# uc-vision/taichi-splatting

Measured on AMD Instinct MI355X. Metric: fwd+bwd Msplats/s, higher is better.
Workload: dtype f32; 1 GPU; config D: 6000000 random 3D gaussians, 2048x2048, SH deg 3, tile 16, fwd+bwd (render_gaussians, loss=image.sum()); n_gaussians=6000000, tile_size=16, sh_degree=3, mode=single, parallelism=single GPU

## Files before the change

taichi_splatting_amd/csrc/frame.hip:

```cpp
#include <cstdlib>
#include <cstring>
#include "common.h"
#include "frame_internal.h"
#include "raster_common.h"

namespace ms {

struct FrameGeom {
  int w_pad, h_pad, tiles_wide, tiles_high, num_tiles, tile_bits, row_begin, row_end;
  size_t es;
};

static FrameGeom frame_geom(const ms_frame_desc* d) {
  FrameGeom g;
  const int ts = d->raster.tile_size;
  g.tiles_wide = (d->image_w + ts - 1) / ts;
  g.tiles_high = (d->image_h + ts - 1) / ts;
  g.w_pad = g.tiles_wide * ts;
  g.h_pad = g.tiles_high * ts;
  g.num_tiles = g.tiles_wide * g.tiles_high;
  int bits = 1;
  while ((1ll << bits) < (long long)g.num_tiles) ++bits;
  g.tile_bits = bits;
  g.row_begin = d->tile_row_begin < 0 ? 0 : d->tile_row_begin;
  g.row_end = d->tile_row_end > g.tiles_high ? g.tiles_high : d->tile_row_end;
  g.es = d->dtype == MS_F64 ? 8 : 4;
  return g;
}

static int check_desc(const ms_frame_desc* d, const char* who) {
  if (!d) { set_error("%s: desc is null", who); return MS_ERR_BAD_ARG; }
  if (d->struct_size != sizeof(ms_frame_desc) || MS_ABI_GENERATION(d->abi_version) != MS_ABI_GENERATION(MS_VERSION)) {
    set_error("%s: ms_frame_desc of another ABI (struct_size %u, abi_version %u; this library: %u, %d) — set desc.struct_size = "
              "sizeof(ms_frame_desc) and desc.abi_version = MS_VERSION of the include/mi355_splat.h you compile against",
              who, d->struct_size, d->abi_version, (unsigned)sizeof(ms_frame_desc), MS_VERSION);
    return MS_ERR_ABI;
  }
  if (d->split_long_runs < 0 || d->split_seg_len < 0) { set_error("%s: negative split parameter", who); return MS_ERR_BAD_ARG; }
  if (d->n < 0 || d->k_capacity < 0) { set_error("%s: negative size", who); return MS_ERR_BAD_ARG; }
  if (d->n >= (1ll << 31) || d->k_capacity >= (1ll << 31)) { set_error("%s: sizes are int32 indexes (< 2^31)", who); return MS_ERR_BAD_ARG; }
  if (d->image_w <= 0 || d->image_h <= 0) { set_error("%s: bad image size", who); return MS_ERR_BAD_ARG; }
  if (d->dtype != MS_F32 && d->dtype != MS_F64) { set_error("%s: dtype must be MS_F32 or MS_F64", who); return MS_ERR_BAD_ARG; }
  const int ts = d->raster.tile_size;
  if (ts != 8 && ts != 16 && ts != 32) { set_error("%s: tile_size must be 8, 16 or 32 (got %d)", who, ts); return MS_ERR_UNSUPPORTED; }
  if (d->f < 1 || d->f > 4) { set_error("%s: 1..4 colour channels (got %d)", who, d->f); return MS_ERR_UNSUPPORTED; }
  if (d->sh_degree < -1 || d->sh_degree > 3) { set_error("%s: SH degree must be in [0, 3]", who); return MS_ERR_BAD_ARG; }
  if (d->mapper != MS_MAPPER_DIRECT && d->mapper != MS_MAPPER_PRESORT) { set_error("%s: mapper must be MS_MAPPER_DIRECT or MS_MAPPER_PRESORT (got %d)", who, d->mapper); return MS_ERR_BAD_ARG; }
  if (d->projected_input && d->sh_degree >= 0) { set_error("%s: projected input carries colours, not SH", who); return MS_ERR_BAD_ARG; }
  if (d->depth16) {
    const FrameGeom g = frame_geom(d);
    if (g.num_tiles > 65536) { set_error("%s: use_depth16 keys hold a 16 bit tile id: too many tiles", who); return MS_ERR_BAD_ARG; }
  }
  return 0;
}

static bool frame_uses_rows(const ms_frame_desc* d) {
  static const bool on = [] { const char* e = getenv("MS_SPLAT_ROWS"); return e && e[0] == '1'; }();
  return on && !d->projected_input && d->n > 0 && raster_uses_splat_rows(&d->raster, d->f, d->dtype);
}

static bool frame_uses_split(const ms_frame_desc* d) {
  return d->split_long_runs != 0 && d->n > 0 && d->k_capacity > 0 && raster_uses_splat_rows(&d->raster, d->f, d->dtype);
}
static SplitParams frame_split_params(const ms_frame_desc* d) {
  return split_params(d->raster.tile_size, d->split_long_runs, d->split_seg_len);
}

static int check_inputs(const ms_frame_inputs* in, const char* who) {
  if (!in) { set_error("%s: inputs are null", who); return MS_ERR_BAD_ARG; }
  if (in->struct_size != sizeof(ms_frame_inputs)) {
    set_error("%s: ms_frame_inputs of another ABI (struct_size %u, this library: %u)", who, in->struct_size, (unsigned)sizeof(ms_frame_inputs));
    return MS_ERR_ABI;
  }
  return 0;
}

static int check_grads(const ms_frame_grads* g, const char* who) {
  if (!g) { set_error("%s: grads are null", who); return MS_ERR_BAD_ARG; }
  if (g->struct_size != sizeof(ms_frame_grads)) {
    set_error("%s: ms_frame_grads of another ABI (struct_size %u, this library: %u)", who, g->struct_size, (unsigned)sizeof(ms_frame_grads));
    return MS_ERR_ABI;
  }
  return 0;
}

struct Carve {
  size_t off = 0;
  size_t take(size_t bytes) { const size_t o = off; off += align_up(bytes > 0 ? bytes : 1, 256); return o; }
};

static void frame_layout(const ms_frame_desc* d, ms_frame_layout* L) {
  const FrameGeom g = frame_geom(d);
  const size_t n = (size_t)d->n, k = (size_t)d->k_capacity;
  const bool own_points = !d->projected_input;
  Carve keep_n, scratch_n, keep_k, scratch_k;
  L->points7 = keep_n.take(own_points ? n * 7 * g.es : 0);
  L->depth = keep_n.take(own_points ? n * g.es : 0);
  L->colours = keep_n.take(d->sh_degree >= 0 ? n * d->f * g.es : 0);
  L->camera_position = keep_n.take(4 * g.es);
  L->counters = keep_n.take(8 * sizeof(int32_t));
  L->tile_ranges = keep_n.take((size_t)g.num_tiles * 2 * sizeof(int32_t));
  L->splat_rows = keep_n.take(frame_uses_rows(d) ? n * SPLAT_ROW * sizeof(float) : 0);
  L->keep_n_bytes = keep_n.off;

  L->sorted_keys = scratch_n.take(n * 4);
  L->order = scratch_n.take(n * 4);
  L->counts = scratch_n.take(n * 4);
  L->cum = scratch_n.take((n + 1) * 4);
  L->ordered_points = scratch_n.take(n * 7 * 4);
  L->points7_f32 = scratch_n.take(d->dtype == MS_F64 ? n * 7 * 4 : 0);
  const size_t t1 = sort_tmp_size(d->n, 4, true), t2 = scan_tmp_size(d->n);
  L->tmp_n = scratch_n.take(t1 > t2 ? t1 : t2);
  L->scratch_n_bytes = scratch_n.off;

  L->overlap_to_point = keep_k.take(k * 4);
  L->split_scratch = keep_k.take(frame_uses_split(d) ? split_scratch_bytes(d->k_capacity, d->raster.tile_size, frame_split_params(d)) : 0);
  L->keep_k_bytes = keep_k.off;

  L->keys = scratch_k.take(k * 8);
  L->values = scratch_k.take(k * 4);
  L->keys_sorted = scratch_k.take(k * 8);
  L->tmp_k = scratch_k.take(sort_tmp_size(d->k_capacity, 8));
  L->scratch_k_bytes = scratch_k.off;
}

template <typename T>
__global__ void __launch_bounds__(256)
frame_prepare_kernel(int32_t* __restrict__ counters, int32_t capacity, const T* __restrict__ Tcw, T* __restrict__ cam_out,
                     int32_t* __restrict__ ranges, int64_t range_words) {
  const int64_t i = (int64_t)blockIdx.x * blockDim.x + threadIdx.x;
  if (i < range_words) ranges[i] = 0;
  if (i == 0) {
    const int32_t k = counters[0];
    const bool ok = k >= 0 && k <= capacity;
    counters[1] = ok ? k : 0;
    counters[2] = ok ? 0 : 1;
    counters[3] = 0;
    counters[4] = 0;
    counters[5] = 0;
    if (cam_out) camera_position_solve(Tcw, cam_out);
  }
}

__global__ void __launch_bounds__(256)
f64_to_f32_kernel(const double* __restrict__ in, float* __restrict__ out, int64_t count) {
  const int64_t i = (int64_t)blockIdx.x * blockDim.x + threadIdx.x;
  if (i < count) out[i] = (float)in[i];
}

static bool mapper_presort(const ms_frame_desc& d) {
  static const int forced = [] {
    const char* e = getenv("MS_MAPPER");
    if (e && strcmp(e, "presort") == 0) return MS_MAPPER_PRESORT;
    if (e && strcmp(e, "direct") == 0) return MS_MAPPER_DIRECT;
    return -1;
  }();
  return (forced >= 0 ? forced : d.mapper) == MS_MAPPER_PRESORT;
}

static bool frame_uses_moments(const ms_frame_desc* d, int deterministic) {
  (void)deterministic;
  return d->dtype == MS_F32 && d->f == 3 && !d->raster.antialias && d->raster.use_alpha_blending;
}

}

using namespace ms;

extern "C" int ms_frame_layout_query(const ms_frame_desc* desc, ms_frame_layout* out) {
  int rc = check_desc(desc, "ms_frame_layout_query");
  if (rc) return rc;
  MS_CHECK_ARG(out != nullptr, "out is null");
  frame_layout(desc, out);
  return 0;
}

extern "C" int ms_frame_uses_moments(const ms_frame_desc* desc, int deterministic) {
  return desc && frame_uses_moments(desc, deterministic) ? 1 : 0;
}

#define MS_TRY(expr)            \
  do {                          \
    const int rc__ = (expr);    \
    if (rc__ != 0) return rc__; \
  } while (0)

static int frame_project_impl(const ms_frame_desc* desc, const ms_frame_inputs* in, void* keep_n, bool projection,
                              bool colours, void* stream, const char* who) {
  const ms_frame_desc& d = *desc;
  if (d.projected_input) { set_error("%s: projected input has no per-gaussian stage", who); return MS_ERR_BAD_ARG; }
  if (d.n == 0) return 0;
  ms_frame_layout L;
  frame_layout(desc, &L);
  char* kn = (char*)keep_n;
  if (!(in->position && in->log_scaling && in->rotation && in->alpha_logit && in->T_camera_world && in->projection)) {
    set_error("%s: null gaussian / camera input", who); return MS_ERR_BAD_ARG;
  }
  if (!in->feature) { set_error("%s: feature is null", who); return MS_ERR_BAD_ARG; }
  float* rows = frame_uses_rows(desc) ? (float*)(kn + L.splat_rows) : nullptr;
  if (projection) {
    if (d.sh_degree >= 0 && colours)
      MS_TRY(ms_camera_position(in->T_camera_world, kn + L.camera_position, d.dtype, stream));
    MS_TRY(project_fwd_launch(in->position, in->log_scaling, in->rotation, in->alpha_logit, in->T_camera_world, in->projection,
                              d.image_w, d.image_h, d.near_plane, d.far_plane, d.blur_cov, d.clamp_margin,
                              d.raster.alpha_threshold, d.n, kn + L.points7, kn + L.depth, nullptr, d.dtype, stream, rows,
                              rows && d.sh_degree < 0 ? in->feature : nullptr));
  }
  if (colours && d.sh_degree >= 0)
    MS_TRY(sh_fwd_inplace_launch(in->feature, in->position, kn + L.depth, kn + L.camera_position, d.n, d.f,
                                 d.sh_degree, kn + L.colours, d.dtype, (hipStream_t)stream, rows));
  return 0;
}

extern "C" int ms_frame_project(const ms_frame_desc* desc, const ms_frame_inputs* in, void* keep_n, void* stream) {
  MS_TRY(check_desc(desc, "ms_frame_project"));
  MS_TRY(check_inputs(in, "ms_frame_project"));
  MS_CHECK_ARG(in && keep_n, "null pointer");
  return frame_project_impl(desc, in, keep_n, true, true, stream, "ms_frame_project");
}

extern "C" int ms_frame_sh_colours(const ms_frame_desc* desc, const ms_frame_inputs* in, void* keep_n, void* stream) {
  MS_TRY(check_desc(desc, "ms_frame_sh_colours"));
  MS_TRY(check_inputs(in, "ms_frame_sh_colours"));
  MS_CHECK_ARG(in && keep_n, "null pointer");
  const ms_frame_desc& d = *desc;
  MS_CHECK_ARG(!d.projected_input && d.sh_degree >= 0, "a frame that evaluates SH colours itself");
  MS_CHECK_ARG(!frame_uses_rows(desc), "the splat-row table is filled on the frame's own stream");
  if (d.n == 0) return 0;
  ms_frame_layout L;
  frame_layout(desc, &L);
  MS_CHECK_ARG(in->T_camera_world != nullptr, "T_camera_world is null");
  MS_TRY(ms_camera_position(in->T_camera_world, (char*)keep_n + L.camera_position, d.dtype, stream));
  return frame_project_impl(desc, in, keep_n, false, true, stream, "ms_frame_sh_colours");
}

extern "C" int ms_frame_project_count(const ms_frame_desc* desc, const ms_frame_inputs* in, void* keep_n,
                                      void* scratch_n, int32_t* k_host, void* k_event, void* stream) {
  MS_TRY(check_desc(desc, "ms_frame_project_count"));
  MS_TRY(check_inputs(in, "ms_frame_project_count"));
  MS_CHECK_ARG(in && keep_n && scratch_n, "null pointer");
  const ms_frame_desc& d = *desc;
  const FrameGeom g = frame_geom(desc);
  ms_frame_layout L;
  frame_layout(desc, &L);
  hipStream_t s = (hipStream_t)stream;
  char* kn = (char*)keep_n;
  char* sn = (char*)scratch_n;
  int32_t* counters = (int32_t*)(kn + L.counters);

  if (d.n == 0) {
    MS_CHECK_HIP(hipMemsetAsync(counters, 0, 8 * sizeof(int32_t), s));
    if (k_host) *k_host = 0;
    if (k_event) MS_CHECK_HIP(hipEventRecord((hipEvent_t)k_event, s));
    return 0;
  }

  const void* points7;
  const void* depth;
  if (!d.projected_input) {
    MS_TRY(frame_project_impl(desc, in, keep_n, true, false, stream, "ms_frame_project_count"));
    points7 = kn + L.points7;
    depth = kn + L.depth;
  } else {
    MS_CHECK_ARG(in->points7 && in->depth && in->colours, "null projected input");
    points7 = in->points7;
    depth = in->depth;
  }

  const float* points_f32 = (const float*)points7;
  if (d.dtype == MS_F64) {
    float* copy = (float*)(sn + L.points7_f32);
    f64_to_f32_kernel<<<dim3((unsigned)div_up(d.n * 7, 256)), dim3(256), 0, s>>>((const double*)points7, copy, d.n * 7);
    points_f32 = copy;
  }

  uint32_t* sorted_keys = (uint32_t*)(sn + L.sorted_keys);
  int32_t* order = (int32_t*)(sn + L.order);
  int32_t* counts = (int32_t*)(sn + L.counts);
  int32_t* cum = (int32_t*)(sn + L.cum);
  const int cull = d.projected_input ? 0 : 1;
  if (mapper_presort(d)) {
    depth_argsort_launch(depth, d.n, d.depth16, d.near_plane > 0.0 ? d.near_plane : 0.0, d.far_plane, d.dtype, cull,
                         sorted_keys, order, sn + L.tmp_n, s);
    tile_count_launch(points_f32, order, cull ? sorted_keys : nullptr, d.n, g.w_pad, g.h_pad, d.raster.tile_size,
                      (float)d.raster.alpha_threshold, g.row_begin, g.row_end, counts, (float*)(sn + L.ordered_points), s);
  } else {
    tile_count_direct_launch(points_f32, cull ? depth : nullptr, d.dtype, d.n, g.w_pad, g.h_pad, d.raster.tile_size,
                             (float)d.raster.alpha_threshold, g.row_begin, g.row_end, counts, s);
  }
  exclusive_scan_launch(counts, d.n, cum, k_host, sn + L.tmp_n, s, counters);
  MS_CHECK_LAUNCH();
  if (k_event) MS_CHECK_HIP(hipEventRecord((hipEvent_t)k_event, s));
  return 0;
}

extern "C" int ms_frame_map_raster(const ms_frame_desc* desc, const ms_frame_inputs* in, void* keep_n, void* scratch_n,
                                   void* keep_k, void* scratch_k, void* out_image, void* out_alpha,
                                   void* out_visibility, void* stream) {
  MS_TRY(check_desc(desc, "ms_frame_map_raster"));
  MS_TRY(check_inputs(in, "ms_frame_map_raster"));
  MS_CHECK_ARG(in && keep_n && scratch_n && out_image && out_alpha, "null pointer");
  const ms_frame_desc& d = *desc;
  const FrameGeom g = frame_geom(desc);
  ms_frame_layout L;
  frame_layout(desc, &L);
  hipStream_t s = (hipStream_t)stream;
  char* kn = (char*)keep_n;
  char* sn = (char*)scratch_n;
  char* kk = (char*)keep_k;
  char* sk = (char*)scratch_k;
  int32_t* counters = (int32_t*)(kn + L.counters);
  int32_t* ranges = (int32_t*)(kn + L.tile_ranges);
  int32_t* o2p = (int32_t*)(kk + L.overlap_to_point);
  const bool colours_elsewhere = !d.projected_input && d.sh_degree >= 0 && in->colours_ready_event != nullptr;

  {
    const bool want_cam = !d.projected_input && d.sh_degree >= 0 && d.n > 0 && !colours_elsewhere;
    if (want_cam) MS_CHECK_ARG(in->T_camera_world != nullptr, "T_camera_world is null");
    const int64_t words = (int64_t)g.num_tiles * 2;
    const dim3 grid((unsigned)(words > 0 ? div_up(words, 256) : 1)), block(256);
    if (d.dtype == MS_F64)
      frame_prepare_kernel<double><<<grid, block, 0, s>>>(counters, (int32_t)d.k_capacity, (const double*)in->T_camera_world,
                                                          want_cam ? (double*)(kn + L.camera_position) : nullptr, ranges, words);
    else
      frame_prepare_kernel<float><<<grid, block, 0, s>>>(counters, (int32_t)d.k_capacity, (const float*)in->T_camera_world,
                                                         want_cam ? (float*)(kn + L.camera_position) : nullptr, ranges, words);
  }
  if (!d.projected_input && !colours_elsewhere) MS_TRY(frame_project_impl(desc, in, keep_n, false, true, stream, "ms_frame_map_raster"));
  if (d.n > 0 && d.k_capacity > 0) {
    MS_CHECK_ARG(keep_k && scratch_k, "null overlap buffers");
    int32_t* values = (int32_t*)(sk + L.values);
    if (mapper_presort(d)) {
      uint32_t* keys = (uint32_t*)(sk + L.keys);
      uint32_t* keys_sorted = (uint32_t*)(sk + L.keys_sorted);
      tile_emit_ordered_launch((const float*)(sn + L.ordered_points), (const int32_t*)(sn + L.order),
                               (const int32_t*)(sn + L.cum), d.n, g.w_pad, g.h_pad, d.raster.tile_size,
                               (float)d.raster.alpha_threshold, g.row_begin, g.row_end, counters + 1, keys, values, s);
      sort_pairs_u32_dev_launch(keys, values, keys_sorted, o2p, d.k_capacity, counters + 1, g.tile_bits, sk + L.tmp_k, s);
      MS_TRY(find_ranges_dev_launch(keys_sorted, d.k_capacity, counters + 1, g.num_tiles, ranges, s, true));
    } else {
      uint64_t* keys = (uint64_t*)(sk + L.keys);
      uint64_t* keys_sorted = (uint64_t*)(sk + L.keys_sorted);
      const void* depth = d.projected_input ? in->depth : (const void*)(kn + L.depth);
      const float* points_f32 = d.dtype == MS_F64 ? (const float*)(sn + L.points7_f32)
                                                  : (const float*)(d.projected_input ? in->points7 : (const void*)(kn + L.points7));
      tile_emit_direct_launch(points_f32, depth, d.dtype, (const int32_t*)(sn + L.cum), d.n, g.w_pad, g.h_pad,
                              d.raster.tile_size, (float)d.raster.alpha_threshold, g.row_begin, g.row_end, d.depth16,
                              d.near_plane > 0.0 ? d.near_plane : 0.0, d.far_plane, counters + 1, keys, values, s);
      sort_pairs_u64_dev_launch(keys, values, keys_sorted, o2p, d.k_capacity, counters + 1, 32, 32 + g.tile_bits,
                                sk + L.tmp_k, s);
      MS_TRY(find_ranges_u64_dev_launch(keys_sorted, d.k_capacity, counters + 1, g.num_tiles, ranges, s));
      const int64_t first_tile = (int64_t)g.row_begin * g.tiles_wide;
      const int64_t strip_tiles = (int64_t)(g.row_end > g.row_begin ? g.row_end - g.row_begin : 0) * g.tiles_wide;
      tile_depth_sort_launch(ranges + 2 * first_tile, strip_tiles, keys_sorted, o2p, keys, s, counters + 3, in->longest_run_host);
    }
  }
  MS_CHECK_LAUNCH();

  const void* points7 = d.projected_input ? in->points7 : (const void*)(kn + L.points7);
  const void* colours = d.sh_degree >= 0 ? (const void*)(kn + L.colours) : (d.projected_input ? in->colours : in->feature);
  MS_CHECK_ARG(d.n == 0 || colours != nullptr, "colours are null");
  SplitScratch split{};
  const bool cut = frame_uses_split(desc) && keep_k != nullptr;
  if (cut) split = split_scratch_carve(kk + L.split_scratch, d.k_capacity, d.raster.tile_size, frame_split_params(desc));
  if (in->colours_ready_event) MS_CHECK_HIP(hipStreamWaitEvent(s, (hipEvent_t)in->colours_ready_event, 0));
  return raster_fwd_launch(points7, colours, frame_uses_rows(desc) ? (const float*)(kn + L.splat_rows) : nullptr, ranges, o2p,
                           d.image_w, d.image_h, d.f, &d.raster, out_image, out_alpha, out_visibility, g.row_begin, g.row_end,
                           d.dtype, stream, cut ? &split : nullptr, in->longest_run_host);
}

extern "C" int ms_frame_backward(const ms_frame_desc* desc, const ms_frame_inputs* in, void* keep_n, void* keep_k,
                                 const ms_frame_grads* gr, void* stream) {
  MS_TRY(check_desc(desc, "ms_frame_backward"));
  MS_TRY(check_inputs(in, "ms_frame_backward"));
  MS_TRY(check_grads(gr, "ms_frame_backward"));
  MS_CHECK_ARG(in && keep_n && gr, "null pointer");
  MS_CHECK_ARG(gr->stage == MS_BACKWARD_GAUSSIANS || (gr->image && gr->grad_image), "null image / grad_image");
  const ms_frame_desc& d = *desc;
  const FrameGeom g = frame_geom(desc);
  ms_frame_layout L;
  frame_layout(desc, &L);
  hipStream_t s = (hipStream_t)stream;
  char* kn = (char*)keep_n;
  char* kk = (char*)keep_k;
  const int32_t* ranges = (const int32_t*)(kn + L.tile_ranges);
  const int32_t* o2p = (const int32_t*)(kk + L.overlap_to_point);
  const void* points7 = d.projected_input ? in->points7 : (const void*)(kn + L.points7);
  const void* depth = d.projected_input ? in->depth : (const void*)(kn + L.depth);
  const void* colours = d.sh_degree >= 0 ? (const void*)(kn + L.colours) : (d.projected_input ? in->colours : in->feature);
  if (d.n == 0) return 0;

  const bool given = gr->stage == MS_BACKWARD_GAUSSIANS;
  const bool raster_only = gr->stage == MS_BACKWARD_RASTER || d.projected_input;
  const bool moments = !given && frame_uses_moments(desc, gr->deterministic);
  MS_CHECK_ARG(!gr->grad_image_broadcast || (!given && moments), "grad_image_broadcast: moments path only (float32 RGB, plain pdf)");
  MS_CHECK_ARG(gr->boundary_form == MS_BOUNDARY_AXIS_SIGMA || gr->boundary_form == MS_BOUNDARY_COVARIANCE, "boundary_form");
  MS_CHECK_ARG(gr->boundary_form == 0 || given || (moments && gr->stage == MS_BACKWARD_RASTER),
               "MS_BOUNDARY_COVARIANCE rows: MS_BACKWARD_GAUSSIANS, or MS_BACKWARD_RASTER on the moments path");
  if (gr->boundary_stride != 0) {
    MS_CHECK_ARG(gr->boundary_stride >= 7 + d.f && d.dtype == MS_F32, "boundary_stride: rows of >= 7 + f floats, float32 frames");
    MS_CHECK_ARG(given || (moments && raster_only), "boundary_stride: MS_BACKWARD_GAUSSIANS, or MS_BACKWARD_RASTER on the moments path");
  }
  if (given) {
    MS_CHECK_ARG(!d.projected_input, "projected input has no per-gaussian backward");
    if (gr->gather_world > 0)
      MS_CHECK_ARG(gr->gather_rows && gr->gather_slots && gr->gather_route && gr->boundary_stride >= 7 + d.f && d.dtype == MS_F32,
                   "gathered boundary gradients: rows, slots, route, boundary_stride >= 7 + f, float32");
    else
      MS_CHECK_ARG(gr->grad_points7 != nullptr, "grad_points7 is null");
  } else if (moments) {
    MS_CHECK_ARG(gr->moments != nullptr, "moments is null");
    SplitScratch split{};
    const bool cut = frame_uses_split(desc) && keep_k != nullptr;
    if (cut) split = split_scratch_carve(kk + L.split_scratch, d.k_capacity, d.raster.tile_size, frame_split_params(desc));
    MS_TRY(raster_bwd_moments_launch(points7, colours, ranges, o2p, gr->image, gr->grad_image, d.image_w, d.image_h, &d.raster,
                                     (float*)gr->moments, gr->deterministic, gr->fixed_exp, g.row_begin, g.row_end,
                                     gr->grad_image_broadcast, s,
                                     frame_uses_rows(desc) ? (const float*)(kn + L.splat_rows) : nullptr,
                                     cut ? &split : nullptr));
    if (raster_only)
      return moments_finalize_rezero_launch((const float*)points7, (float*)gr->moments, gr->deterministic, gr->fixed_exp,
                                            d.n, (float*)gr->grad_points7, (float*)gr->grad_colours,
                                            d.raster.compute_point_heuristic ? (float*)gr->point_heuristic : nullptr, s,
                                            gr->boundary_stride, d.projected_input && gr->stage != MS_BACKWARD_RASTER ? 0 : gr->boundary_form);
  } else {
    MS_CHECK_ARG(gr->grad_points7 || gr->grad_colours, "no gradient accumulator");
    MS_TRY(ms_raster_bwd(points7, colours, ranges, o2p, gr->image, gr->grad_image, d.image_w, d.image_h, d.f, &d.raster,
                         gr->grad_points7, gr->grad_colours, d.raster.compute_point_heuristic ? gr->point_heuristic : nullptr,
                         g.row_begin, g.row_end, d.dtype, stream));
    if (raster_only) return 0;
  }

  GaussianBwdArgs a{};
  a.dtype = d.dtype;
  a.n = d.n;
  a.position = in->position; a.log_scaling = in->log_scaling; a.rotation = in->rotation; a.alpha_logit = in->alpha_logit;
  a.T_camera_world = in->T_camera_world; a.projection = in->projection;
  a.image_w = d.image_w; a.image_h = d.image_h;
  a.blur_cov = d.blur_cov; a.clamp_margin = d.clamp_margin;
  a.depth = depth;
  if (moments) {
    a.moments = gr->moments; a.deterministic = gr->deterministic; a.fixed_exp = gr->fixed_exp;
    a.store_points7 = gr->grad_points7; a.store_colours = gr->grad_colours;
    a.point_heuristic = d.raster.compute_point_heuristic ? gr->point_heuristic : nullptr;
    a.point_visibility = d.raster.compute_point_heuristic ? gr->point_visibility : nullptr;
  } else {
    a.grad_points7 = gr->grad_points7; a.grad_colours = gr->grad_colours;
    a.boundary_stride = gr->boundary_stride;
    a.boundary_cov = given ? gr->boundary_form : 0;
    if (given && gr->gather_world > 0) {
      a.gather_world = gr->gather_world; a.gather_rows = gr->gather_rows;
      a.gather_slots = gr->gather_slots; a.gather_route = gr->gather_route;
    }
  }
  a.extra_points7 = gr->extra_points7; a.extra_depth = gr->extra_depth; a.extra_colours = gr->extra_colours;
  a.sh_degree = d.sh_degree; a.f = d.f;
  a.camera_position = kn + L.camera_position; a.colours = colours;
  a.grad_position = gr->grad_position; a.grad_log_scaling = gr->grad_log_scaling; a.grad_rotation = gr->grad_rotation;
  a.grad_alpha_logit = gr->grad_alpha_logit; a.grad_feature = gr->grad_feature; a.grad_camera = gr->grad_camera;
  return gaussian_bwd_launch(a, s);
}
```

taichi_splatting_amd/csrc/frame_internal.h:

```cpp
#pragma once
#include "common.h"

namespace ms {

constexpr uint32_t CULLED_DEPTH_KEY = 0xffffffffu;

template <typename T>
__device__ inline void camera_position_solve(const T* __restrict__ m, T* __restrict__ out) {
#pragma clang fp contract(off)
  double a[4][5];
  for (int r = 0; r < 4; ++r) {
    for (int c = 0; c < 4; ++c) a[r][c] = (double)m[r * 4 + c];
    a[r][4] = r == 3 ? 1.0 : 0.0;
  }
  for (int col = 0; col < 4; ++col) {
    int piv = col;
    for (int r = col + 1; r < 4; ++r)
      if (fabs(a[r][col]) > fabs(a[piv][col])) piv = r;
    for (int c = 0; c < 5; ++c) { const double t = a[col][c]; a[col][c] = a[piv][c]; a[piv][c] = t; }
    const double inv = 1.0 / a[col][col];
    for (int c = 0; c < 5; ++c) a[col][c] *= inv;
    for (int r = 0; r < 4; ++r) {
      if (r == col) continue;
      const double fct = a[r][col];
      for (int c = 0; c < 5; ++c) a[r][c] -= fct * a[col][c];
    }
  }
  for (int k = 0; k < 3; ++k) out[k] = (T)a[k][4];
}

size_t scan_tmp_size(int64_t n);
size_t sort_tmp_size(int64_t n, int key_bytes, bool adaptive = false);
void exclusive_scan_launch(const int32_t* in, int64_t n, int32_t* out, int32_t* total_host, void* tmp, hipStream_t s,
                           int32_t* total_copy = nullptr);
void depth_argsort_launch(const void* depth, int64_t n, int depth16, double ndc_near, double ndc_far, int dtype,
                          int cull, uint32_t* out_sorted_keys, int32_t* out_order, char* tmp, hipStream_t s);
void sort_pairs_u32_dev_launch(const uint32_t* keys_in, const int32_t* vals_in, uint32_t* keys_out, int32_t* vals_out,
                               int64_t capacity, const int32_t* n_dev, int end_bit, char* tmp, hipStream_t s);
int find_ranges_dev_launch(const uint32_t* sorted_keys, int64_t capacity, const int32_t* k_dev, int64_t num_tiles,
                           int32_t* out_ranges, hipStream_t s, bool zeroed = false);

void sort_pairs_u64_dev_launch(const uint64_t* keys_in, const int32_t* vals_in, uint64_t* keys_out, int32_t* vals_out,
                               int64_t capacity, const int32_t* n_dev, int begin_bit, int end_bit, char* tmp, hipStream_t s);
int find_ranges_u64_dev_launch(const uint64_t* sorted_keys, int64_t capacity, const int32_t* k_dev, int64_t num_tiles,
                               int32_t* out_ranges, hipStream_t s);

void tile_count_launch(const float* points7, const int32_t* order, const uint32_t* cull_keys, int64_t v, int image_w,
                       int image_h, int tile_size, float alpha_threshold, int row_begin, int row_end,
                       int32_t* out_counts, float* out_ordered, hipStream_t s);
void tile_emit_ordered_launch(const float* ordered_points7, const int32_t* order, const int32_t* cum, int64_t v,
                              int image_w, int image_h, int tile_size, float alpha_threshold, int row_begin,
                              int row_end, const int32_t* k_limit_dev, uint32_t* out_keys, int32_t* out_values,
                              hipStream_t s);

void tile_count_direct_launch(const float* points7, const void* cull_depth, int dtype, int64_t v, int image_w, int image_h,
                              int tile_size, float alpha_threshold, int row_begin, int row_end, int32_t* out_counts,
                              hipStream_t s);
void tile_emit_direct_launch(const float* points7, const void* depth, int dtype, const int32_t* cum, int64_t v, int image_w,
                             int image_h, int tile_size, float alpha_threshold, int row_begin, int row_end, int depth16,
                             double ndc_near, double ndc_far, const int32_t* k_limit_dev, uint64_t* out_keys,
                             int32_t* out_values, hipStream_t s);

void tile_depth_sort_launch(const int32_t* tile_ranges, int64_t num_tiles, uint64_t* sorted_keys, int32_t* overlap_to_point,
                            uint64_t* scratch, hipStream_t s, int32_t* run_stats = nullptr, int32_t* run_host = nullptr);

int project_fwd_launch(const void* position, const void* log_scaling, const void* rotation, const void* alpha_logit,
                       const void* T_camera_world, const void* projection, int image_w, int image_h, double near_plane,
                       double far_plane, double blur_cov, double clamp_margin, double alpha_threshold, int64_t n,
                       void* out_points7, void* out_depth, int32_t* out_flag, int dtype, void* stream, float* splat_rows,
                       const void* colours_in);

int sh_fwd_inplace_launch(const void* params, const void* positions, const void* depth, const void* cam_pos,
                          int64_t n, int f, int degree, void* out, int dtype, hipStream_t s, float* splat_rows = nullptr);

bool raster_uses_splat_rows(const ms_raster_config* cfg, int f, int dtype);
int raster_fwd_launch(const void* points7, const void* features, const float* splat_rows, const int32_t* tile_ranges,
                      const int32_t* overlap_to_point, int image_w, int image_h, int f, const ms_raster_config* cfg,
                      void* out_image, void* out_alpha, void* out_visibility, int tile_row_begin, int tile_row_end,
                      int dtype, void* stream, const struct SplitScratch* split = nullptr, int32_t* long_run_word = nullptr);

int raster_bwd_moments_launch(const void* points7, const void* features, const int32_t* tile_ranges,
                              const int32_t* overlap_to_point, const void* image, const void* grad_image, int image_w,
                              int image_h, const ms_raster_config* cfg, float* moments, int deterministic,
                              const int32_t* fixed_exp, int tile_row_begin, int tile_row_end, int grad_broadcast,
                              hipStream_t s, const float* splat_rows = nullptr, const struct SplitScratch* split = nullptr);
int moments_finalize_rezero_launch(const float* points7, float* moments, int deterministic, const int32_t* fixed_exp,
                                   int64_t n, float* grad_points7, float* grad_features, float* point_heuristic,
                                   hipStream_t s, int row_stride = 0, int covariance_form = 0);

struct GaussianBwdArgs {
  int dtype;
  int64_t n;
  const void *position, *log_scaling, *rotation, *alpha_logit, *T_camera_world, *projection;
  int image_w, image_h;
  double blur_cov, clamp_margin;
  const void* depth;
  void* moments;
  int deterministic;
  const int32_t* fixed_exp;
  const void* grad_points7;
  const void* grad_colours;
  int boundary_cov;
  int boundary_stride;
  int gather_world;
  const void* gather_rows;
  const int32_t *gather_slots, *gather_route;
  const void *extra_points7, *extra_depth, *extra_colours;
  int sh_degree, f;
  const void *camera_position, *colours;
  void *grad_position, *grad_log_scaling, *grad_rotation, *grad_alpha_logit;
  void* grad_feature;
  void* grad_camera;
  void *store_points7, *store_colours;
  void* point_heuristic;
  void* point_visibility;
};
int gaussian_bwd_launch(const GaussianBwdArgs& a, hipStream_t s);

}
```

taichi_splatting_amd/csrc/mapper.hip:

```cpp
#pragma clang fp contract(off)
#include "common.h"
#include "frame_internal.h"

namespace ms {

__device__ __forceinline__ void load_point7(const float* __restrict__ points, int64_t i, float g[7]) {
#pragma unroll
  for (int k = 0; k < 7; ++k) g[k] = points[i * 7 + k];
}


__device__ __forceinline__ float readlane_f(float v, int lane) {
  return __int_as_float(__builtin_amdgcn_readlane(__float_as_int(v), lane));
}
__device__ __forceinline__ ObbQuery wave_broadcast(const ObbQuery& q, int lane) {
  ObbQuery r;
  r.inv00 = readlane_f(q.inv00, lane); r.inv01 = readlane_f(q.inv01, lane);
  r.inv10 = readlane_f(q.inv10, lane); r.inv11 = readlane_f(q.inv11, lane);
  r.rel_min_x = readlane_f(q.rel_min_x, lane); r.rel_min_y = readlane_f(q.rel_min_y, lane);
  r.min_tile_x = __builtin_amdgcn_readlane(q.min_tile_x, lane); r.min_tile_y = __builtin_amdgcn_readlane(q.min_tile_y, lane);
  r.span_x = __builtin_amdgcn_readlane(q.span_x, lane); r.span_y = __builtin_amdgcn_readlane(q.span_y, lane);
  return r;
}
__device__ __forceinline__ unsigned long long wide_span_lanes(const ObbQuery& q, bool valid, int* my_span) {
  const int span = valid && q.span_x > 0 && q.span_y > 0 ? q.span_x * q.span_y : 0;
  *my_span = span;
  const int total = (int)readlane_f(wave_sum_to_lane63((float)span), 63);
  int thr = total / 32;
  thr = thr > 16 ? thr : 16;
  return __ballot(span > thr);
}
template <typename F>
__device__ __forceinline__ void wave_walk_span(const ObbQuery& b, int tile_size, int row_begin, int row_end, F on_hits) {
  const int n = b.span_x * b.span_y, lane = lane_id();
  for (int base = 0; base < n; base += 64) {
    const int idx = base + lane;
    bool hit = false;
    int tu = 0, tv = 0;
    if (idx < n) {
      tv = idx / b.span_x; tu = idx - tv * b.span_x;
      const int ty = b.min_tile_y + tv;
      hit = ty >= row_begin && ty < row_end && obb_test_tile(b, tu, tv, tile_size);
    }
    on_hits(hit, b.min_tile_x + tu, b.min_tile_y + tv);
  }
}
__device__ __forceinline__ int count_span(const ObbQuery& q, bool valid, int tile_size, int row_begin, int row_end) {
  int span;
  unsigned long long wide = wide_span_lanes(q, valid, &span);
  const bool mine_is_wide = (wide >> lane_id()) & 1ull;
  int count = 0;
  if (span > 0 && !mine_is_wide) {
    for (int tv = 0; tv < q.span_y; ++tv) {
      const int ty = q.min_tile_y + tv;
      if (ty < row_begin || ty >= row_end) continue;
      for (int tu = 0; tu < q.span_x; ++tu)
        if (obb_test_tile(q, tu, tv, tile_size)) ++count;
    }
  }
  while (wide != 0) {
    const int src = __builtin_ctzll(wide);
    wide &= wide - 1;
    const ObbQuery b = wave_broadcast(q, src);
    int total = 0;
    wave_walk_span(b, tile_size, row_begin, row_end, [&](bool hit, int, int) { total += __builtin_popcountll(__ballot(hit)); });
    if (lane_id() == src) count = total;
  }
  return count;
}
template <typename F>
__device__ __forceinline__ void emit_span(const ObbQuery& q, bool valid, int64_t first, int tile_size, int row_begin,
                                          int row_end, F emit) {
  int span;
  unsigned long long wide = wide_span_lanes(q, valid, &span);
  const bool mine_is_wide = (wide >> lane_id()) & 1ull;
  if (span > 0 && !mine_is_wide) {
    int64_t o = first;
    for (int tu = 0; tu < q.span_x; ++tu) {
      for (int tv = 0; tv < q.span_y; ++tv) {
        const int ty = q.min_tile_y + tv;
        if (ty < row_begin || ty >= row_end) continue;
        if (obb_test_tile(q, tu, tv, tile_size)) emit(o++, q.min_tile_x + tu, ty, -1);
      }
    }
  }
  while (wide != 0) {
    const int src = __builtin_ctzll(wide);
    wide &= wide - 1;
    const ObbQuery b = wave_broadcast(q, src);
    const int lo = __builtin_amdgcn_readlane((int)(uint32_t)first, src), hi = __builtin_amdgcn_readlane((int)(uint32_t)(first >> 32), src);
    int64_t o = (int64_t)(((uint64_t)(uint32_t)hi << 32) | (uint32_t)lo);
    wave_walk_span(b, tile_size, row_begin, row_end, [&](bool hit, int tx, int ty) {
      const unsigned long long m = __ballot(hit);
      if (hit) emit(o + (int)__builtin_amdgcn_mbcnt_hi((uint32_t)(m >> 32), __builtin_amdgcn_mbcnt_lo((uint32_t)m, 0u)), tx, ty, src);
      o += __builtin_popcountll(m);
    });
  }
}

__global__ void __launch_bounds__(256)
tile_count_kernel(const float* __restrict__ points, const int32_t* __restrict__ order,
                  const uint32_t* __restrict__ cull_keys, int64_t v, int image_w,
                  int image_h, int tile_size, float alpha_threshold, int row_begin, int row_end,
                  int32_t* __restrict__ counts, float* __restrict__ ordered_points) {
  const int64_t i = (int64_t)blockIdx.x * blockDim.x + threadIdx.x;
  const bool valid = i < v && !(cull_keys && cull_keys[i] == CULLED_DEPTH_KEY);
  float g[7] = {0.f, 0.f, 1.f, 0.f, 1.f, 1.f, 0.f};
  if (valid) {
    load_point7(points, order ? (int64_t)order[i] : i, g);
    if (ordered_points) {
#pragma unroll
      for (int k = 0; k < 7; ++k) ordered_points[i * 7 + k] = g[k];
    }
  }
  const ObbQuery q = obb_grid_query(g, image_w, image_h, tile_size, alpha_threshold);
  const int count = count_span(q, valid, tile_size, row_begin, row_end);
  if (i < v) counts[i] = count;
}

template <typename KeyT, int MODE>
__global__ void __launch_bounds__(256)
tile_emit_kernel(const float* __restrict__ points, const float* __restrict__ depth,
                 const int32_t* __restrict__ order, const int32_t* __restrict__ cum, int64_t v,
                 int image_w, int image_h, int tile_size, float alpha_threshold, int row_begin,
                 int row_end, int points_ordered, const int32_t* __restrict__ k_limit,
                 KeyT* __restrict__ keys, int32_t* __restrict__ values) {
  const int64_t i = (int64_t)blockIdx.x * blockDim.x + threadIdx.x;
  if (k_limit && *k_limit == 0) return;
  const bool valid = i < v && !(k_limit && cum[i + 1] == cum[i]);
  const int64_t src = valid ? (order ? (int64_t)order[i] : i) : 0;
  float g[7] = {0.f, 0.f, 1.f, 0.f, 1.f, 1.f, 0.f};
  if (valid) load_point7(points, points_ordered ? i : src, g);
  const ObbQuery q = obb_grid_query(g, image_w, image_h, tile_size, alpha_threshold);
  const int tiles_wide = image_w / tile_size;
  KeyT depth_key = 0;
  if (valid) {
    if (MODE == 1) {
      const float c = fminf(fmaxf(depth[src], 0.0f), 1.0f);
      depth_key = (KeyT)(uint32_t)(c * 65535.0f);
    } else if (MODE == 0) {
      depth_key = (KeyT)__float_as_uint(depth[src]);
    }
  }
  const uint32_t dk_lo = (uint32_t)depth_key, dk_hi = (uint32_t)((uint64_t)depth_key >> 32);
  emit_span(q, valid, valid ? (int64_t)cum[i] : 0, tile_size, row_begin, row_end, [&](int64_t o, int tx, int ty, int from) {
    const int64_t tile_id = (int64_t)tx + (int64_t)ty * tiles_wide;
    KeyT dk = depth_key;
    int32_t who = (int32_t)src;
    if (from >= 0) {
      dk = (KeyT)(((uint64_t)(uint32_t)__builtin_amdgcn_readlane((int)dk_hi, from) << 32) | (uint32_t)__builtin_amdgcn_readlane((int)dk_lo, from));
      who = __builtin_amdgcn_readlane((int32_t)src, from);
    }
    if constexpr (MODE == 2) keys[o] = (KeyT)tile_id;
    else if constexpr (MODE == 1) keys[o] = (KeyT)(dk | ((KeyT)tile_id << 16));
    else keys[o] = (KeyT)(dk | ((KeyT)tile_id << 32));
    values[o] = who;
  });
}

template <typename T>
__global__ void __launch_bounds__(256, 8)
tile_count_direct_kernel(const float* __restrict__ points, const T* __restrict__ cull_depth, int64_t v, int image_w,
                         int image_h, int tile_size, float alpha_threshold, int row_begin, int row_end,
                         int32_t* __restrict__ counts) {
  const int64_t i = (int64_t)blockIdx.x * blockDim.x + threadIdx.x;
  const bool valid = i < v && !(cull_depth && !(cull_depth[i] > T(0)));
  float g[7] = {0.f, 0.f, 1.f, 0.f, 1.f, 1.f, 0.f};
  if (valid) load_point7(points, i, g);
  const ObbQuery q = obb_grid_query(g, image_w, image_h, tile_size, alpha_threshold);
  const int count = count_span(q, valid, tile_size, row_begin, row_end);
  if (i < v) counts[i] = count;
}

template <typename T>
__global__ void __launch_bounds__(256)
tile_emit_direct_kernel(const float* __restrict__ points, const T* __restrict__ depth, const int32_t* __restrict__ cum,
                        int64_t v, int image_w, int image_h, int tile_size, float alpha_threshold, int row_begin,
                        int row_end, int depth16, double near_plane, double far_plane,
                        const int32_t* __restrict__ k_limit, uint64_t* __restrict__ keys, int32_t* __restrict__ values) {
  const int64_t i = (int64_t)blockIdx.x * blockDim.x + threadIdx.x;
  if (k_limit && *k_limit == 0) return;
  const int64_t first = i < v ? (int64_t)cum[i] : 0;
  const bool valid = i < v && cum[i + 1] != first;
  float g[7] = {0.f, 0.f, 1.f, 0.f, 1.f, 1.f, 0.f};
  if (valid) load_point7(points, i, g);
  const ObbQuery q = obb_grid_query(g, image_w, image_h, tile_size, alpha_threshold);
  const int tiles_wide = image_w / tile_size;
  const uint32_t depth_key = valid ? (uint32_t)depth_sort_key(depth[i], depth16, near_plane, far_plane) : 0u;
  emit_span(q, valid, first, tile_size, row_begin, row_end, [&](int64_t o, int tx, int ty, int from) {
    const uint64_t tile_id = (uint64_t)((int64_t)tx + (int64_t)ty * tiles_wide);
    uint32_t dk = depth_key;
    int32_t who = (int32_t)i;
    if (from >= 0) { dk = (uint32_t)__builtin_amdgcn_readlane((int)depth_key, from); who = __builtin_amdgcn_readlane((int32_t)i, from); }
    keys[o] = (tile_id << 32) | dk;
    values[o] = who;
  });
}

template <typename T>
__global__ void __launch_bounds__(256)
depth_keys_kernel(const T* __restrict__ depth, int64_t v, int depth16, double near_plane, double far_plane,
                  uint32_t* __restrict__ keys, int32_t* __restrict__ values) {
  const int64_t i = (int64_t)blockIdx.x * blockDim.x + threadIdx.x;
  if (i >= v) return;
  keys[i] = depth_sort_key(depth[i], depth16, near_plane, far_plane);
  values[i] = (int32_t)i;
}

void tile_count_launch(const float* points7, const int32_t* order, const uint32_t* cull_keys, int64_t v, int image_w,
                       int image_h, int tile_size, float alpha_threshold, int row_begin, int row_end,
                       int32_t* out_counts, float* out_ordered, hipStream_t s) {
  tile_count_kernel<<<dim3((unsigned)div_up(v, 256)), dim3(256), 0, s>>>(
      points7, order, cull_keys, v, image_w, image_h, tile_size, alpha_threshold, row_begin, row_end, out_counts, out_ordered);
}

void tile_emit_ordered_launch(const float* ordered_points7, const int32_t* order, const int32_t* cum, int64_t v,
                              int image_w, int image_h, int tile_size, float alpha_threshold, int row_begin,
                              int row_end, const int32_t* k_limit_dev, uint32_t* out_keys, int32_t* out_values,
                              hipStream_t s) {
  tile_emit_kernel<uint32_t, 2><<<dim3((unsigned)div_up(v, 256)), dim3(256), 0, s>>>(
      ordered_points7, nullptr, order, cum, v, image_w, image_h, tile_size, alpha_threshold, row_begin, row_end, 1,
      k_limit_dev, out_keys, out_values);
}

void tile_count_direct_launch(const float* points7, const void* cull_depth, int dtype, int64_t v, int image_w, int image_h,
                              int tile_size, float alpha_threshold, int row_begin, int row_end, int32_t* out_counts,
                              hipStream_t s) {
  const dim3 grid((unsigned)div_up(v, 256)), block(256);
  if (dtype == MS_F64)
    tile_count_direct_kernel<double><<<grid, block, 0, s>>>(points7, (const double*)cull_depth, v, image_w, image_h, tile_size,
                                                            alpha_threshold, row_begin, row_end, out_counts);
  else
    tile_count_direct_kernel<float><<<grid, block, 0, s>>>(points7, (const float*)cull_depth, v, image_w, image_h, tile_size,
                                                           alpha_threshold, row_begin, row_end, out_counts);
}

void tile_emit_direct_launch(const float* points7, const void* depth, int dtype, const int32_t* cum, int64_t v, int image_w,
                             int image_h, int tile_size, float alpha_threshold, int row_begin, int row_end, int depth16,
                             double ndc_near, double ndc_far, const int32_t* k_limit_dev, uint64_t* out_keys,
                             int32_t* out_values, hipStream_t s) {
  const dim3 grid((unsigned)div_up(v, 256)), block(256);
  if (dtype == MS_F64)
    tile_emit_direct_kernel<double><<<grid, block, 0, s>>>(points7, (const double*)depth, cum, v, image_w, image_h, tile_size,
                                                           alpha_threshold, row_begin, row_end, depth16, ndc_near, ndc_far,
                                                           k_limit_dev, out_keys, out_values);
  else
    tile_emit_direct_kernel<float><<<grid, block, 0, s>>>(points7, (const float*)depth, cum, v, image_w, image_h, tile_size,
                                                          alpha_threshold, row_begin, row_end, depth16, ndc_near, ndc_far,
                                                          k_limit_dev, out_keys, out_values);
}

}

using namespace ms;

extern "C" int ms_depth_sort_keys(const void* depth, int64_t v, int depth16, double ndc_near, double ndc_far,
                                  uint32_t* out_keys, int32_t* out_values, int dtype, void* stream) {
  MS_CHECK_ARG(v >= 0, "v < 0");
  MS_CHECK_ARG(dtype == MS_F32 || dtype == MS_F64, "dtype must be MS_F32 or MS_F64");
  if (v == 0) return 0;
  MS_CHECK_ARG(depth && out_keys && out_values, "null pointer");
  const dim3 grid((unsigned)div_up(v, 256)), block(256);
  if (dtype == MS_F32)
    depth_keys_kernel<float><<<grid, block, 0, (hipStream_t)stream>>>((const float*)depth, v, depth16, ndc_near, ndc_far, out_keys, out_values);
  else
    depth_keys_kernel<double><<<grid, block, 0, (hipStream_t)stream>>>((const double*)depth, v, depth16, ndc_near, ndc_far, out_keys, out_values);
  MS_CHECK_LAUNCH();
  return 0;
}

extern "C" int ms_tile_count(const float* points7, const int32_t* order, int64_t v, int image_w, int image_h, int tile_size,
                             float alpha_threshold, int tile_row_begin, int tile_row_end,
                             int32_t* out_counts, float* out_ordered_points7, void* stream) {
  MS_CHECK_ARG(v >= 0, "v < 0");
  MS_CHECK_ARG(tile_size > 0 && image_w > 0 && image_h > 0, "bad image/tile size");
  MS_CHECK_ARG(image_w % tile_size == 0 && image_h % tile_size == 0, "image size must be padded to the tile size");
  if (v == 0) return 0;
  MS_CHECK_ARG(points7 && out_counts, "null pointer");
  tile_count_kernel<<<dim3((unsigned)div_up(v, 256)), dim3(256), 0, (hipStream_t)stream>>>(
      points7, order, nullptr, v, image_w, image_h, tile_size, alpha_threshold, tile_row_begin, tile_row_end, out_counts, out_ordered_points7);
  MS_CHECK_LAUNCH();
  return 0;
}

extern "C" int ms_tile_emit(const float* points7, const float* depth, const int32_t* order, const int32_t* cum,
                            int64_t v, int image_w, int image_h, int tile_size, float alpha_threshold,
                            int tile_row_begin, int tile_row_end, int key_mode, int points_are_ordered,
                            void* out_keys, int32_t* out_values, void* stream) {
  MS_CHECK_ARG(v >= 0, "v < 0");
  MS_CHECK_ARG(key_mode >= 0 && key_mode <= 2, "key_mode must be 0 (tile|depth32), 1 (tile|depth16) or 2 (tile only)");
  MS_CHECK_ARG(tile_size > 0 && image_w > 0 && image_h > 0, "bad image/tile size");
  MS_CHECK_ARG(image_w % tile_size == 0 && image_h % tile_size == 0, "image size must be padded to the tile size");
  if (key_mode == 1) {
    const int64_t tiles = (int64_t)(image_w / tile_size) * (image_h / tile_size);
    MS_CHECK_ARG(tiles <= 65536, "use_depth16 keys hold a 16 bit tile id: too many tiles");
  }
  if (v == 0) return 0;
  MS_CHECK_ARG(points7 && cum && out_keys && out_values, "null pointer");
  MS_CHECK_ARG(key_mode == 2 || depth, "depth is null");
  const dim3 block(256), grid((unsigned)div_up(v, 256));
  hipStream_t s = (hipStream_t)stream;
#define MS_EMIT(KeyT, MODE) tile_emit_kernel<KeyT, MODE><<<grid, block, 0, s>>>(points7, depth, order, cum, v, image_w, image_h, tile_size, alpha_threshold, tile_row_begin, tile_row_end, points_are_ordered, nullptr, (KeyT*)out_keys, out_values)
  if (key_mode == 0) MS_EMIT(uint64_t, 0);
  else if (key_mode == 1) MS_EMIT(uint32_t, 1);
  else MS_EMIT(uint32_t, 2);
#undef MS_EMIT
  MS_CHECK_LAUNCH();
  return 0;
}

extern "C" int ms_tile_emit_keys64(const float* points7, const void* depth, int depth_dtype, const int32_t* cum, int64_t v,
                                   int image_w, int image_h, int tile_size, float alpha_threshold, int tile_row_begin,
                                   int tile_row_end, int depth16, double ndc_near, double ndc_far, uint64_t* out_keys,
                                   int32_t* out_values, void* stream) {
  MS_CHECK_ARG(v >= 0, "v < 0");
  MS_CHECK_ARG(depth_dtype == MS_F32 || depth_dtype == MS_F64, "depth_dtype must be MS_F32 or MS_F64");
  MS_CHECK_ARG(tile_size > 0 && image_w > 0 && image_h > 0, "bad image/tile size");
  MS_CHECK_ARG(image_w % tile_size == 0 && image_h % tile_size == 0, "image size must be padded to the tile size");
  if (depth16) {
    const int64_t tiles = (int64_t)(image_w / tile_size) * (image_h / tile_size);
    MS_CHECK_ARG(tiles <= 65536, "use_depth16 keys hold a 16 bit tile id: too many tiles");
  }
  if (v == 0) return 0;
  MS_CHECK_ARG(points7 && depth && cum && out_keys && out_values, "null pointer");
  tile_emit_direct_launch(points7, depth, depth_dtype, cum, v, image_w, image_h, tile_size, alpha_threshold, tile_row_begin,
                          tile_row_end, depth16, ndc_near > 0.0 ? ndc_near : 0.0, ndc_far, nullptr, out_keys, out_values,
                          (hipStream_t)stream);
  MS_CHECK_LAUNCH();
  return 0;
}
```

taichi_splatting_amd/csrc/scan_sort.hip:

```cpp
#include "common.h"
#include "frame_internal.h"

namespace ms {

constexpr int SCAN_THREADS = 256;
constexpr int SCAN_ITEMS = 16;
constexpr int SCAN_TILE = SCAN_THREADS * SCAN_ITEMS;

__device__ __forceinline__ int block_exclusive_scan(int v, int* lds , int* block_total) {
  const int lane = lane_id(), wave = threadIdx.x >> 6;
  int incl = v;
#pragma unroll
  for (int off = 1; off < 64; off <<= 1) {
    const int t = __shfl_up(incl, off, 64);
    if (lane >= off) incl += t;
  }
  if (lane == 63) lds[wave] = incl;
  __syncthreads();
  int wave_off = 0, total = 0;
#pragma unroll
  for (int w = 0; w < SCAN_THREADS / 64; ++w) {
    const int s = lds[w];
    if (w < wave) wave_off += s;
    total += s;
  }
  __syncthreads();
  *block_total = total;
  return wave_off + incl - v;
}

__device__ __forceinline__ void load_items(const int32_t* __restrict__ in, int64_t base, int64_t n, int (&vals)[SCAN_ITEMS]) {
  if (base + SCAN_ITEMS <= n && (reinterpret_cast<uintptr_t>(in + base) & 15) == 0) {
    const int4* p = reinterpret_cast<const int4*>(in + base);
#pragma unroll
    for (int q = 0; q < SCAN_ITEMS / 4; ++q) {
      const int4 v = p[q];
      vals[4 * q] = v.x; vals[4 * q + 1] = v.y; vals[4 * q + 2] = v.z; vals[4 * q + 3] = v.w;
    }
  } else {
#pragma unroll
    for (int k = 0; k < SCAN_ITEMS; ++k) vals[k] = base + k < n ? in[base + k] : 0;
  }
}

__device__ __forceinline__ void store_items(int32_t* __restrict__ out, int64_t base, int64_t n, const int (&vals)[SCAN_ITEMS]) {
  if (base + SCAN_ITEMS <= n && (reinterpret_cast<uintptr_t>(out + base) & 15) == 0) {
    int4* p = reinterpret_cast<int4*>(out + base);
#pragma unroll
    for (int q = 0; q < SCAN_ITEMS / 4; ++q) p[q] = make_int4(vals[4 * q], vals[4 * q + 1], vals[4 * q + 2], vals[4 * q + 3]);
  } else {
#pragma unroll
    for (int k = 0; k < SCAN_ITEMS; ++k) if (base + k < n) out[base + k] = vals[k];
  }
}

__global__ void __launch_bounds__(SCAN_THREADS)
scan_block_sums_kernel(const int32_t* __restrict__ in, int64_t n, int32_t* __restrict__ block_sums) {
  __shared__ int lds[4];
  const int64_t base = (int64_t)blockIdx.x * SCAN_TILE + (int64_t)threadIdx.x * SCAN_ITEMS;
  int items[SCAN_ITEMS];
  load_items(in, base, n, items);
  int s = 0;
#pragma unroll
  for (int k = 0; k < SCAN_ITEMS; ++k) s += items[k];
  int total;
  block_exclusive_scan(s, lds, &total);
  if (threadIdx.x == 0) block_sums[blockIdx.x] = total;
}

__global__ void __launch_bounds__(SCAN_THREADS)
scan_spine_kernel(int32_t* __restrict__ block_sums, int64_t num_blocks, int32_t* __restrict__ total_out,
                  int32_t* __restrict__ total_host, int32_t* __restrict__ total_copy = nullptr) {
  __shared__ int lds[4];
  int carry = 0;
  for (int64_t base = 0; base < num_blocks; base += SCAN_THREADS) {
    const int64_t i = base + threadIdx.x;
    const int v = i < num_blocks ? block_sums[i] : 0;
    int total;
    const int ex = block_exclusive_scan(v, lds, &total);
    if (i < num_blocks) block_sums[i] = carry + ex;
    carry += total;
  }
  if (threadIdx.x == 0) {
    *total_out = carry;
    if (total_copy) *total_copy = carry;
    if (total_host) *total_host = carry;
  }
}

__global__ void __launch_bounds__(SCAN_THREADS)
scan_downsweep_kernel(const int32_t* __restrict__ in, int64_t n, const int32_t* __restrict__ block_offsets,
                      int32_t* __restrict__ out) {
  __shared__ int lds[4];
  const int64_t base = (int64_t)blockIdx.x * SCAN_TILE + (int64_t)threadIdx.x * SCAN_ITEMS;
  int vals[SCAN_ITEMS];
  load_items(in, base, n, vals);
  int s = 0;
#pragma unroll
  for (int k = 0; k < SCAN_ITEMS; ++k) s += vals[k];
  int total;
  int prefix = block_exclusive_scan(s, lds, &total) + block_offsets[blockIdx.x];
#pragma unroll
  for (int k = 0; k < SCAN_ITEMS; ++k) {
    const int v = vals[k];
    vals[k] = prefix;
    prefix += v;
  }
  store_items(out, base, n, vals);
}

constexpr int64_t SCAN_SELF_MAX_BLOCKS = 8192;

__global__ void __launch_bounds__(SCAN_THREADS)
scan_downsweep_self_kernel(const int32_t* __restrict__ in, int64_t n, const int32_t* __restrict__ block_sums,
                           int32_t* __restrict__ out, int32_t* __restrict__ total_host,
                           int32_t* __restrict__ total_copy = nullptr) {
  __shared__ int lds[4];
  int before = 0;
  for (int j = threadIdx.x; j < (int)blockIdx.x; j += SCAN_THREADS) before += block_sums[j];
  int block_prefix;
  block_exclusive_scan(before, lds, &block_prefix);

  const int64_t base = (int64_t)blockIdx.x * SCAN_TILE + (int64_t)threadIdx.x * SCAN_ITEMS;
  int vals[SCAN_ITEMS];
  load_items(in, base, n, vals);
  int s = 0;
#pragma unroll
  for (int k = 0; k < SCAN_ITEMS; ++k) s += vals[k];
  int total;
  int prefix = block_exclusive_scan(s, lds, &total) + block_prefix;
#pragma unroll
  for (int k = 0; k < SCAN_ITEMS; ++k) {
    const int v = vals[k];
    vals[k] = prefix;
    prefix += v;
  }
  store_items(out, base, n, vals);
  if (blockIdx.x == gridDim.x - 1 && threadIdx.x == 0) {
    out[n] = block_prefix + total;
    if (total_copy) *total_copy = block_prefix + total;
    if (total_host) *total_host = block_prefix + total;
  }
}

static size_t scan_tmp_bytes(int64_t n) { return align_up((size_t)div_up(n > 0 ? n : 1, SCAN_TILE) * sizeof(int32_t), 256); }

static int exclusive_scan_i32(const int32_t* in, int64_t n, int32_t* out, int32_t* total_host, void* tmp,
                              hipStream_t s, int32_t* total_copy = nullptr) {
  const int64_t blocks = div_up(n, SCAN_TILE);
  int32_t* block_sums = (int32_t*)tmp;
  scan_block_sums_kernel<<<dim3((unsigned)blocks), dim3(SCAN_THREADS), 0, s>>>(in, n, block_sums);
  if (blocks <= SCAN_SELF_MAX_BLOCKS) {
    scan_downsweep_self_kernel<<<dim3((unsigned)blocks), dim3(SCAN_THREADS), 0, s>>>(in, n, block_sums, out, total_host, total_copy);
    return 0;
  }
  scan_spine_kernel<<<dim3(1), dim3(SCAN_THREADS), 0, s>>>(block_sums, blocks, out + n, total_host, total_copy);
  scan_downsweep_kernel<<<dim3((unsigned)blocks), dim3(SCAN_THREADS), 0, s>>>(in, n, block_sums, out);
  return 0;
}

constexpr int RS_THREADS = 256;
constexpr int RS_WAVES = RS_THREADS / 64;
constexpr int RS_ROUNDS = 16;
constexpr int RS_WAVE_ITEMS = RS_ROUNDS * 64;
constexpr int RS_TILE = RS_THREADS * RS_ROUNDS;
constexpr int RS_RADIX = 256;

template <typename KeyT>
__device__ __forceinline__ unsigned key_digit(KeyT k, int shift, unsigned mask) {
  return (unsigned)(k >> shift) & mask;
}

template <typename KeyT> struct PlainPairs {
  const KeyT* keys;
  const int32_t* vals;
  __device__ __forceinline__ KeyT key(int64_t i) const { return keys[i]; }
  __device__ __forceinline__ int32_t val(int64_t i) const { return vals[i]; }
};
template <typename T> struct DepthPairs {
  const T* depth;
  int depth16;
  double near_plane, far_plane;
  int cull;
  __device__ __forceinline__ uint32_t key(int64_t i) const {
    const T d = depth[i];
    if (cull && !(d > T(0))) return CULLED_DEPTH_KEY;
    return depth_sort_key(d, depth16, near_plane, far_plane);
  }
  __device__ __forceinline__ int32_t val(int64_t i) const { return (int32_t)i; }
};

template <typename KeyT, typename Source, bool VARY = false>
__device__ __forceinline__ void upsweep_block(const Source src, int64_t n, int shift, unsigned mask,
                                              int32_t* __restrict__ hist, int64_t num_blocks,
                                              uint32_t* __restrict__ blk_or = nullptr, uint32_t* __restrict__ blk_and = nullptr) {
  constexpr int RS_COPIES = 4;
  __shared__ unsigned cnt[RS_WAVES][RS_COPIES][RS_RADIX];
  __shared__ unsigned s_or, s_and;
  for (int i = threadIdx.x; i < RS_WAVES * RS_COPIES * RS_RADIX; i += RS_THREADS) (&cnt[0][0][0])[i] = 0;
  if (VARY && threadIdx.x == 0) { s_or = 0u; s_and = ~0u; }
  __syncthreads();
  const int wave = threadIdx.x >> 6, lane = lane_id();
  unsigned* mine = cnt[wave][lane & (RS_COPIES - 1)];
  const int64_t base = (int64_t)blockIdx.x * RS_TILE + (int64_t)wave * RS_WAVE_ITEMS + lane;
  unsigned v_or = 0u, v_and = ~0u;
  if ((int64_t)(blockIdx.x + 1) * RS_TILE <= n) {
    KeyT k[RS_ROUNDS];
#pragma unroll
    for (int j = 0; j < RS_ROUNDS; ++j) k[j] = src.key(base + j * 64);
#pragma unroll
    for (int j = 0; j < RS_ROUNDS; ++j) {
      atomicAdd(&mine[key_digit(k[j], shift, mask)], 1u);
      if (VARY && (uint32_t)k[j] != 0xffffffffu) { v_or |= (uint32_t)k[j]; v_and &= (uint32_t)k[j]; }
    }
  } else {
#pragma unroll 4
    for (int j = 0; j < RS_ROUNDS; ++j) {
      const int64_t i = base + j * 64;
      if (i < n) {
        const KeyT key = src.key(i);
        atomicAdd(&mine[key_digit(key, shift, mask)], 1u);
        if (VARY && (uint32_t)key != 0xffffffffu) { v_or |= (uint32_t)key; v_and &= (uint32_t)key; }
      }
    }
  }
  if (VARY) {
#pragma unroll
    for (int off = 32; off >= 1; off >>= 1) { v_or |= __shfl_xor(v_or, off); v_and &= __shfl_xor(v_and, off); }
    if (lane == 0) { atomicOr(&s_or, v_or); atomicAnd(&s_and, v_and); }
  }
  __syncthreads();
  for (int d = threadIdx.x; d < RS_RADIX; d += RS_THREADS) {
    unsigned t = 0;
#pragma unroll
    for (int w = 0; w < RS_WAVES; ++w)
#pragma unroll
      for (int c = 0; c < RS_COPIES; ++c) t += cnt[w][c][d];
    hist[(int64_t)d * num_blocks + blockIdx.x] = (int32_t)t;
  }
  if (VARY && threadIdx.x == 0) { blk_or[blockIdx.x] = s_or; blk_and[blockIdx.x] = s_and; }
}

template <typename KeyT, typename Source>
__global__ void __launch_bounds__(RS_THREADS)
radix_upsweep_kernel(const Source src, int64_t n, const int32_t* __restrict__ n_dev, int shift, unsigned mask,
                     int32_t* __restrict__ hist, int64_t num_blocks) {
  if (n_dev) n = *n_dev;
  upsweep_block<KeyT, Source>(src, n, shift, mask, hist, num_blocks);
}

__device__ __forceinline__ void row_scan_body(int32_t* __restrict__ hist, int64_t num_blocks, int32_t* __restrict__ digit_totals) {
  __shared__ int lds[4];
  int32_t* row = hist + (int64_t)blockIdx.x * num_blocks;
  int carry = 0;
  for (int64_t base = 0; base < num_blocks; base += SCAN_TILE) {
    const int64_t mine = base + (int64_t)threadIdx.x * SCAN_ITEMS;
    int vals[SCAN_ITEMS];
    load_items(row, mine, num_blocks, vals);
    int s = 0;
#pragma unroll
    for (int k = 0; k < SCAN_ITEMS; ++k) s += vals[k];
    int total;
    int prefix = carry + block_exclusive_scan(s, lds, &total);
#pragma unroll
    for (int k = 0; k < SCAN_ITEMS; ++k) {
      const int v = vals[k];
      vals[k] = prefix;
      prefix += v;
    }
    store_items(row, mine, num_blocks, vals);
    carry += total;
  }
  if (threadIdx.x == 0) digit_totals[blockIdx.x] = carry;
}

__global__ void __launch_bounds__(SCAN_THREADS)
radix_row_scan_kernel(int32_t* __restrict__ hist, int64_t num_blocks, int32_t* __restrict__ digit_totals) {
  row_scan_body(hist, num_blocks, digit_totals);
}

template <typename KeyT> struct DownsweepShared {
  unsigned cnt[RS_WAVES][RS_RADIX];
  int scan[4];
  unsigned digit_shift[RS_RADIX];
  KeyT keys[RS_TILE];
  int32_t vals[RS_TILE];
};

template <typename KeyT, bool FULL, typename Source>
__device__ __forceinline__ void downsweep_block(DownsweepShared<KeyT>& sh, const Source src, KeyT* __restrict__ keys_out,
                                                int32_t* __restrict__ vals_out, int64_t n, int shift, unsigned mask,
                                                const int32_t* __restrict__ hist_scanned,
                                                const int32_t* __restrict__ digit_totals, int64_t num_blocks) {
  for (int i = threadIdx.x; i < RS_WAVES * RS_RADIX; i += RS_THREADS) (&sh.cnt[0][0])[i] = 0;
  __syncthreads();

  const int wave = threadIdx.x >> 6, lane = lane_id();
  const int64_t base = (int64_t)blockIdx.x * RS_TILE + (int64_t)wave * RS_WAVE_ITEMS + lane;
  const unsigned long long lanes_below = (1ull << lane) - 1ull;

  KeyT k[RS_ROUNDS];
  int32_t v[RS_ROUNDS];
  unsigned rank[RS_ROUNDS];

#pragma unroll
  for (int j = 0; j < RS_ROUNDS; ++j) {
    const int64_t i = base + j * 64;
    const bool valid = FULL || i < n;
    k[j] = valid ? src.key(i) : (KeyT)0;
    v[j] = valid ? src.val(i) : 0;
  }

#pragma unroll
  for (int j = 0; j < RS_ROUNDS; ++j) {
    const int64_t i = base + j * 64;
    const bool valid = FULL || i < n;
    const unsigned d = key_digit(k[j], shift, mask);
    const unsigned long long valid_lanes = FULL ? ~0ull : __ballot(valid);
    unsigned peers_lo = (unsigned)valid_lanes, peers_hi = (unsigned)(valid_lanes >> 32);
#pragma unroll
    for (int b = 0; b < 8; ++b) {
      const int m = __builtin_amdgcn_sbfe((int)d, b, 1);
      const unsigned long long bal = __ballot(m != 0);
      peers_lo &= ~((unsigned)bal ^ (unsigned)m);
      peers_hi &= ~((unsigned)(bal >> 32) ^ (unsigned)m);
    }
    const unsigned long long peers = ((unsigned long long)peers_hi << 32) | peers_lo;
    const unsigned below = (unsigned)__popcll(peers & lanes_below);
    unsigned prev = 0;
    if (valid) {
      prev = sh.cnt[wave][d];
    }
    __builtin_amdgcn_wave_barrier();
    if (valid && below == 0) sh.cnt[wave][d] = prev + (unsigned)__popcll(peers);
    __builtin_amdgcn_wave_barrier();
    rank[j] = prev + below;
  }
  __syncthreads();

  {
    const int d = threadIdx.x;
    unsigned total = 0;
#pragma unroll
    for (int w = 0; w < RS_WAVES; ++w) total += sh.cnt[w][d];
    int block_total;
    const unsigned local = (unsigned)block_exclusive_scan((int)total, sh.scan, &block_total);
    unsigned run = local;
#pragma unroll
    for (int w = 0; w < RS_WAVES; ++w) {
      const unsigned c = sh.cnt[w][d];
      sh.cnt[w][d] = run;
      run += c;
    }
    int all_items;
    const unsigned digit_base = (unsigned)block_exclusive_scan(digit_totals[d], sh.scan, &all_items);
    sh.digit_shift[d] = digit_base + (unsigned)hist_scanned[(int64_t)d * num_blocks + blockIdx.x] - local;
  }
  __syncthreads();

#pragma unroll
  for (int j = 0; j < RS_ROUNDS; ++j) {
    const int64_t i = base + j * 64;
    if (FULL || i < n) {
      const unsigned d = key_digit(k[j], shift, mask);
      const unsigned lp = sh.cnt[wave][d] + rank[j];
      sh.keys[lp] = k[j];
      sh.vals[lp] = v[j];
    }
  }
  __syncthreads();
  const int64_t block_base = (int64_t)blockIdx.x * RS_TILE;
  const int block_items = FULL ? RS_TILE : (int)(n - block_base);
#pragma unroll
  for (int j = 0; j < RS_ROUNDS; ++j) {
    const int idx = (int)threadIdx.x + j * RS_THREADS;
    if (FULL || idx < block_items) {
      const KeyT key = sh.keys[idx];
      const unsigned d = key_digit(key, shift, mask);
      const int64_t pos = (int64_t)(unsigned)(sh.digit_shift[d] + (unsigned)idx);
      keys_out[pos] = key;
      vals_out[pos] = sh.vals[idx];
    }
  }
}

template <typename KeyT, typename Source>
__global__ void __launch_bounds__(RS_THREADS)
radix_downsweep_kernel(const Source src,
                       KeyT* __restrict__ keys_out, int32_t* __restrict__ vals_out, int64_t n,
                       const int32_t* __restrict__ n_dev, int shift,
                       unsigned mask, const int32_t* __restrict__ hist_scanned,
                       const int32_t* __restrict__ digit_totals, int64_t num_blocks) {
  __shared__ DownsweepShared<KeyT> sh;
  if (n_dev) {
    n = *n_dev;
    if ((int64_t)blockIdx.x * RS_TILE >= n) return;
  }
  if ((int64_t)(blockIdx.x + 1) * RS_TILE <= n)
    downsweep_block<KeyT, true>(sh, src, keys_out, vals_out, n, shift, mask, hist_scanned, digit_totals, num_blocks);
  else
    downsweep_block<KeyT, false>(sh, src, keys_out, vals_out, n, shift, mask, hist_scanned, digit_totals, num_blocks);
}

template <typename KeyT>
__global__ void __launch_bounds__(256)
copy_pairs_kernel(const KeyT* __restrict__ ki, const int32_t* __restrict__ vi, KeyT* __restrict__ ko,
                  int32_t* __restrict__ vo, int64_t n) {
  const int64_t i = (int64_t)blockIdx.x * blockDim.x + threadIdx.x;
  if (i < n) { ko[i] = ki[i]; vo[i] = vi[i]; }
}

struct SortTmp {
  size_t hist_off, scan_off, keys_off, vals_off, keys2_off, vals2_off, vary_off, total;
};

static SortTmp sort_tmp_layout(int64_t n, int key_bytes, bool adaptive = false) {
  const int64_t blocks = div_up(n > 0 ? n : 1, RS_TILE);
  SortTmp t;
  size_t off = 0;
  t.hist_off = off; off += align_up((size_t)(RS_RADIX * blocks + 1) * sizeof(int32_t), 256);
  t.scan_off = off; off += align_up((size_t)RS_RADIX * sizeof(int32_t), 256);
  t.keys_off = off; off += align_up((size_t)n * key_bytes, 256);
  t.vals_off = off; off += align_up((size_t)n * sizeof(int32_t), 256);
  t.keys2_off = t.vals2_off = t.vary_off = off;
  if (adaptive) {
    t.keys2_off = off; off += align_up((size_t)n * key_bytes, 256);
    t.vals2_off = off; off += align_up((size_t)n * sizeof(int32_t), 256);
    t.vary_off = off; off += align_up((size_t)(64 + 2 * blocks) * sizeof(uint32_t), 256);
  }
  t.total = off;
  return t;
}

template <typename KeyT, typename First>
static int radix_sort_passes(const First first, KeyT* keys_out, int32_t* vals_out, int64_t n, int begin_bit, int end_bit,
                             char* tmp, hipStream_t s, const int32_t* n_dev = nullptr) {
  const int64_t blocks = div_up(n, RS_TILE);
  const SortTmp lay = sort_tmp_layout(n, sizeof(KeyT));
  int32_t* hist = (int32_t*)(tmp + lay.hist_off);
  int32_t* digit_totals = (int32_t*)(tmp + lay.scan_off);
  KeyT* keys_alt = (KeyT*)(tmp + lay.keys_off);
  int32_t* vals_alt = (int32_t*)(tmp + lay.vals_off);
  const int passes = (end_bit - begin_bit + 7) / 8;
  const dim3 grid((unsigned)blocks), block(RS_THREADS);
  PlainPairs<KeyT> src{nullptr, nullptr};
  const int total_bits = end_bit - begin_bit, base_bits = total_bits / passes, wide = total_bits % passes;
  int shift = begin_bit;
  for (int p = 0; p < passes; shift += base_bits + (p < wide ? 1 : 0), ++p) {
    const int bits = base_bits + (p < wide ? 1 : 0);
    const unsigned mask = (1u << bits) - 1u;
    const bool to_out = ((passes - 1 - p) % 2) == 0;
    KeyT* dst_k = to_out ? keys_out : keys_alt;
    int32_t* dst_v = to_out ? vals_out : vals_alt;
    if (p == 0) radix_upsweep_kernel<KeyT, First><<<grid, block, 0, s>>>(first, n, n_dev, shift, mask, hist, blocks);
    else radix_upsweep_kernel<KeyT, PlainPairs<KeyT>><<<grid, block, 0, s>>>(src, n, n_dev, shift, mask, hist, blocks);
    radix_row_scan_kernel<<<dim3(RS_RADIX), dim3(SCAN_THREADS), 0, s>>>(hist, blocks, digit_totals);
    if (p == 0) radix_downsweep_kernel<KeyT, First><<<grid, block, 0, s>>>(first, dst_k, dst_v, n, n_dev, shift, mask, hist, digit_totals, blocks);
    else radix_downsweep_kernel<KeyT, PlainPairs<KeyT>><<<grid, block, 0, s>>>(src, dst_k, dst_v, n, n_dev, shift, mask, hist, digit_totals, blocks);
    src = PlainPairs<KeyT>{dst_k, dst_v};
  }
  return 0;
}

struct AdaptiveBufs {
  uint32_t *k_alt[2], *k_out;
  int32_t *v_alt[2], *v_out;
  uint32_t* vary;
};

__device__ __forceinline__ void adaptive_route(uint32_t vary, int p, int passes, bool& active, int& k, bool& last) {
  unsigned m = 1u;
  for (int q = 1; q < passes; ++q)
    if ((vary >> (8 * q)) & 0xffu) m |= 1u << q;
  active = ((m >> p) & 1u) != 0u;
  k = __popc(m & ((1u << p) - 1u));
  last = (m >> (p + 1)) == 0u;
}

template <typename First>
__global__ void __launch_bounds__(RS_THREADS)
depth_upsweep_first_kernel(const First first, AdaptiveBufs b, int64_t n, int32_t* __restrict__ hist, int64_t num_blocks) {
  upsweep_block<uint32_t, First, true>(first, n, 0, 0xffu, hist, num_blocks, b.vary + 64, b.vary + 64 + num_blocks);
}

__global__ void __launch_bounds__(RS_THREADS)
depth_upsweep_kernel(AdaptiveBufs b, int p, int passes, int64_t n, int32_t* __restrict__ hist, int64_t num_blocks) {
  bool active, last; int k;
  adaptive_route(b.vary[0], p, passes, active, k, last);
  if (!active) return;
  upsweep_block<uint32_t, PlainPairs<uint32_t>>(PlainPairs<uint32_t>{b.k_alt[(k - 1) & 1], b.v_alt[(k - 1) & 1]}, n, 8 * p, 0xffu, hist, num_blocks);
}

__global__ void __launch_bounds__(SCAN_THREADS)
depth_row_scan_kernel(int32_t* __restrict__ hist, int64_t num_blocks, int32_t* __restrict__ digit_totals, AdaptiveBufs b,
                      int p, int passes) {
  if (p > 0) {
    bool active, last; int k;
    adaptive_route(b.vary[0], p, passes, active, k, last);
    if (!active) return;
  }
  row_scan_body(hist, num_blocks, digit_totals);
  if (p == 0 && blockIdx.x == 0) {
    __shared__ unsigned s_or, s_and;
    if (threadIdx.x == 0) { s_or = 0u; s_and = ~0u; }
    __syncthreads();
    unsigned v_or = 0u, v_and = ~0u;
    for (int64_t i = threadIdx.x; i < num_blocks; i += blockDim.x) { v_or |= b.vary[64 + i]; v_and &= b.vary[64 + num_blocks + i]; }
    atomicOr(&s_or, v_or); atomicAnd(&s_and, v_and);
    __syncthreads();
    if (threadIdx.x == 0) b.vary[0] = s_or >= s_and && s_or != 0u ? (s_or ^ s_and) : 0u;
  }
}

template <typename First>
__global__ void __launch_bounds__(RS_THREADS)
depth_downsweep_first_kernel(const First first, AdaptiveBufs b, int passes, int64_t n,
                             const int32_t* __restrict__ hist_scanned, const int32_t* __restrict__ digit_totals, int64_t num_blocks) {
  __shared__ DownsweepShared<uint32_t> sh;
  bool active, last; int k;
  adaptive_route(b.vary[0], 0, passes, active, k, last);
  uint32_t* ko = last ? b.k_out : b.k_alt[0];
  int32_t* vo = last ? b.v_out : b.v_alt[0];
  if ((int64_t)(blockIdx.x + 1) * RS_TILE <= n) downsweep_block<uint32_t, true>(sh, first, ko, vo, n, 0, 0xffu, hist_scanned, digit_totals, num_blocks);
  else downsweep_block<uint32_t, false>(sh, first, ko, vo, n, 0, 0xffu, hist_scanned, digit_totals, num_blocks);
}

__global__ void __launch_bounds__(RS_THREADS)
depth_downsweep_kernel(AdaptiveBufs b, int p, int passes, int64_t n, const int32_t* __restrict__ hist_scanned,
                       const int32_t* __restrict__ digit_totals, int64_t num_blocks) {
  __shared__ DownsweepShared<uint32_t> sh;
  bool active, last; int k;
  adaptive_route(b.vary[0], p, passes, active, k, last);
  if (!active) return;
  uint32_t* ko = last ? b.k_out : b.k_alt[k & 1];
  int32_t* vo = last ? b.v_out : b.v_alt[k & 1];
  const PlainPairs<uint32_t> src{b.k_alt[(k - 1) & 1], b.v_alt[(k - 1) & 1]};
  if ((int64_t)(blockIdx.x + 1) * RS_TILE <= n) downsweep_block<uint32_t, true>(sh, src, ko, vo, n, 8 * p, 0xffu, hist_scanned, digit_totals, num_blocks);
  else downsweep_block<uint32_t, false>(sh, src, ko, vo, n, 8 * p, 0xffu, hist_scanned, digit_totals, num_blocks);
}

template <typename First>
static int radix_sort_depth_adaptive(const First first, uint32_t* keys_out, int32_t* vals_out, int64_t n, int end_bit,
                                     char* tmp, hipStream_t s) {
  const int64_t blocks = div_up(n, RS_TILE);
  const SortTmp lay = sort_tmp_layout(n, 4, true);
  int32_t* hist = (int32_t*)(tmp + lay.hist_off);
  int32_t* digit_totals = (int32_t*)(tmp + lay.scan_off);
  AdaptiveBufs b;
  b.k_alt[0] = (uint32_t*)(tmp + lay.keys_off); b.v_alt[0] = (int32_t*)(tmp + lay.vals_off);
  b.k_alt[1] = (uint32_t*)(tmp + lay.keys2_off); b.v_alt[1] = (int32_t*)(tmp + lay.vals2_off);
  b.k_out = keys_out; b.v_out = vals_out;
  b.vary = (uint32_t*)(tmp + lay.vary_off);
  const int passes = (end_bit + 7) / 8;
  const dim3 grid((unsigned)blocks), block(RS_THREADS);
  for (int p = 0; p < passes; ++p) {
    if (p == 0) depth_upsweep_first_kernel<First><<<grid, block, 0, s>>>(first, b, n, hist, blocks);
    else depth_upsweep_kernel<<<grid, block, 0, s>>>(b, p, passes, n, hist, blocks);
    depth_row_scan_kernel<<<dim3(RS_RADIX), dim3(SCAN_THREADS), 0, s>>>(hist, blocks, digit_totals, b, p, passes);
    if (p == 0) depth_downsweep_first_kernel<First><<<grid, block, 0, s>>>(first, b, passes, n, hist, digit_totals, blocks);
    else depth_downsweep_kernel<<<grid, block, 0, s>>>(b, p, passes, n, hist, digit_totals, blocks);
  }
  return 0;
}

template <typename KeyT>
static int radix_sort_pairs_impl(const KeyT* keys_in, const int32_t* vals_in, KeyT* keys_out,
                                 int32_t* vals_out, int64_t n, int begin_bit, int end_bit, char* tmp,
                                 hipStream_t s) {
  if ((end_bit - begin_bit + 7) / 8 == 0) {
    copy_pairs_kernel<KeyT><<<dim3((unsigned)div_up(n, 256)), dim3(256), 0, s>>>(keys_in, vals_in, keys_out, vals_out, n);
    return 0;
  }
  return radix_sort_passes<KeyT>(PlainPairs<KeyT>{keys_in, vals_in}, keys_out, vals_out, n, begin_bit, end_bit, tmp, s);
}

__global__ void __launch_bounds__(256)
segmented_rank_sort_kernel(const int32_t* __restrict__ keys_in, const int32_t* __restrict__ vals_in,
                           int32_t* __restrict__ keys_out, int32_t* __restrict__ vals_out,
                           const int64_t* __restrict__ starts, const int64_t* __restrict__ ends) {
  const int64_t b = starts[blockIdx.x], e = ends[blockIdx.x];
  for (int64_t i = b + threadIdx.x; i < e; i += blockDim.x) {
    const int32_t k = keys_in[i];
    int64_t r = 0;
    for (int64_t j = b; j < e; ++j) {
      const int32_t kj = keys_in[j];
      r += (kj < k) || (kj == k && j < i);
    }
    keys_out[b + r] = k;
    vals_out[b + r] = vals_in[i];
  }
}

template <typename KeyT>
__global__ void __launch_bounds__(256)
find_ranges_kernel(const KeyT* __restrict__ keys, int64_t k, const int32_t* __restrict__ k_dev, int shift,
                   int64_t num_tiles, int32_t* __restrict__ ranges) {
  const int64_t i = (int64_t)blockIdx.x * blockDim.x + threadIdx.x;
  if (k_dev) k = *k_dev;
  if (i >= k) return;
  const int64_t tile = (int64_t)(keys[i] >> shift);
  const int64_t next = (i + 1 < k) ? (int64_t)(keys[i + 1] >> shift) : -1;
  if (i == 0 && tile < num_tiles) ranges[tile * 2 + 0] = 0;
  if (tile != next) {
    if (tile < num_tiles) ranges[tile * 2 + 1] = (int32_t)(i + 1);
    if (next >= 0 && next < num_tiles) ranges[next * 2 + 0] = (int32_t)(i + 1);
  }
}

__global__ void __launch_bounds__(256)
find_ranges4_kernel(const uint32_t* __restrict__ keys, int64_t capacity, const int32_t* __restrict__ k_dev,
                    int64_t num_tiles, int32_t* __restrict__ ranges) {
  const int64_t i0 = ((int64_t)blockIdx.x * blockDim.x + threadIdx.x) * 4;
  const int64_t k = k_dev ? (int64_t)*k_dev : capacity;
  if (i0 >= k) return;
  uint32_t t[5];
  if (i0 + 4 < k) {
    const uint4 v = *reinterpret_cast<const uint4*>(keys + i0);
    t[0] = v.x; t[1] = v.y; t[2] = v.z; t[3] = v.w; t[4] = keys[i0 + 4];
  } else {
#pragma unroll
    for (int j = 0; j < 5; ++j) t[j] = i0 + j < k ? keys[i0 + j] : 0xffffffffu;
  }
  if (i0 == 0 && (int64_t)t[0] < num_tiles) ranges[(int64_t)t[0] * 2 + 0] = 0;
#pragma unroll
  for (int j = 0; j < 4; ++j) {
    const int64_t i = i0 + j;
    if (i >= k) break;
    const int64_t tile = t[j], next = (i + 1 < k) ? (int64_t)t[j + 1] : -1;
    if (tile != next) {
      if (tile < num_tiles) ranges[tile * 2 + 1] = (int32_t)(i + 1);
      if (next >= 0 && next < num_tiles) ranges[next * 2 + 0] = (int32_t)(i + 1);
    }
  }
}

__global__ void __launch_bounds__(256)
find_ranges2_u64_kernel(const uint64_t* __restrict__ keys, int64_t capacity, const int32_t* __restrict__ k_dev,
                        int64_t num_tiles, int32_t* __restrict__ ranges) {
  const int64_t i0 = ((int64_t)blockIdx.x * blockDim.x + threadIdx.x) * 2;
  const int64_t k = k_dev ? (int64_t)*k_dev : capacity;
  uint32_t t0 = 0xffffffffu, t1 = 0xffffffffu;
  if (i0 + 1 < k) {
    const uint4 a = *reinterpret_cast<const uint4*>(keys + i0);
    t0 = a.y; t1 = a.w;
  } else if (i0 < k) {
    t0 = (uint32_t)(keys[i0] >> 32);
  }
  uint32_t t2 = (uint32_t)__shfl_down((int)t0, 1);
  if ((threadIdx.x & 63) == 63) t2 = i0 + 2 < k ? (uint32_t)(keys[i0 + 2] >> 32) : 0xffffffffu;
  if (i0 >= k) return;
  if (i0 == 0 && (int64_t)t0 < num_tiles) ranges[(int64_t)t0 * 2 + 0] = 0;
  const uint32_t t[3] = {t0, t1, t2};
#pragma unroll
  for (int j = 0; j < 2; ++j) {
    const int64_t i = i0 + j;
    if (i >= k) break;
    const int64_t tile = t[j], next = (i + 1 < k) ? (int64_t)t[j + 1] : -1;
    if (tile != next) {
      if (tile < num_tiles) ranges[tile * 2 + 1] = (int32_t)(i + 1);
      if (next >= 0 && next < num_tiles) ranges[next * 2 + 0] = (int32_t)(i + 1);
    }
  }
}

size_t scan_tmp_size(int64_t n) { return scan_tmp_bytes(n); }
size_t sort_tmp_size(int64_t n, int key_bytes, bool adaptive) { return sort_tmp_layout(n, key_bytes, adaptive).total; }

void exclusive_scan_launch(const int32_t* in, int64_t n, int32_t* out, int32_t* total_host, void* tmp, hipStream_t s,
                           int32_t* total_copy) {
  exclusive_scan_i32(in, n, out, total_host, tmp, s, total_copy);
}

void depth_argsort_launch(const void* depth, int64_t n, int depth16, double ndc_near, double ndc_far, int dtype,
                          int cull, uint32_t* out_sorted_keys, int32_t* out_order, char* tmp, hipStream_t s) {
  const int end_bit = depth16 ? 16 : 32;
  if (dtype == MS_F32)
    radix_sort_depth_adaptive(DepthPairs<float>{(const float*)depth, depth16, ndc_near, ndc_far, cull}, out_sorted_keys, out_order, n, end_bit, tmp, s);
  else
    radix_sort_depth_adaptive(DepthPairs<double>{(const double*)depth, depth16, ndc_near, ndc_far, cull}, out_sorted_keys, out_order, n, end_bit, tmp, s);
}

void sort_pairs_u32_dev_launch(const uint32_t* keys_in, const int32_t* vals_in, uint32_t* keys_out, int32_t* vals_out,
                               int64_t capacity, const int32_t* n_dev, int end_bit, char* tmp, hipStream_t s) {
  radix_sort_passes<uint32_t>(PlainPairs<uint32_t>{keys_in, vals_in}, keys_out, vals_out, capacity, 0, end_bit, tmp, s, n_dev);
}

int find_ranges_dev_launch(const uint32_t* sorted_keys, int64_t capacity, const int32_t* k_dev, int64_t num_tiles,
                           int32_t* out_ranges, hipStream_t s, bool zeroed) {
  if (num_tiles > 0 && !zeroed) MS_CHECK_HIP(hipMemsetAsync(out_ranges, 0, (size_t)num_tiles * 2 * sizeof(int32_t), s));
  if (capacity > 0)
    find_ranges4_kernel<<<dim3((unsigned)div_up(capacity, 1024)), dim3(256), 0, s>>>(sorted_keys, capacity, k_dev, num_tiles, out_ranges);
  return 0;
}

void sort_pairs_u64_dev_launch(const uint64_t* keys_in, const int32_t* vals_in, uint64_t* keys_out, int32_t* vals_out,
                               int64_t capacity, const int32_t* n_dev, int begin_bit, int end_bit, char* tmp, hipStream_t s) {
  radix_sort_passes<uint64_t>(PlainPairs<uint64_t>{keys_in, vals_in}, keys_out, vals_out, capacity, begin_bit, end_bit, tmp, s, n_dev);
}

int find_ranges_u64_dev_launch(const uint64_t* sorted_keys, int64_t capacity, const int32_t* k_dev, int64_t num_tiles,
                               int32_t* out_ranges, hipStream_t s) {
  if (capacity > 0)
    find_ranges2_u64_kernel<<<dim3((unsigned)div_up(capacity, 512)), dim3(256), 0, s>>>(sorted_keys, capacity, k_dev, num_tiles, out_ranges);
  return 0;
}

}

using namespace ms;

extern "C" int ms_exclusive_scan_i32(const int32_t* in, int64_t n, int32_t* out, int32_t* total_host,
                                     void* tmp, size_t* tmp_bytes, void* stream) {
  MS_CHECK_ARG(n >= 0, "n < 0");
  MS_CHECK_ARG(tmp_bytes != nullptr, "tmp_bytes is null");
  const size_t need = scan_tmp_bytes(n);
  if (tmp == nullptr) { *tmp_bytes = need; return 0; }
  if (*tmp_bytes < need) { set_error("ms_exclusive_scan_i32: tmp too small (%zu < %zu)", *tmp_bytes, need); return MS_ERR_TMP_TOO_SMALL; }
  MS_CHECK_ARG(out != nullptr, "out is null");
  MS_CHECK_ARG(n == 0 || in != nullptr, "in is null");
  if (n == 0) {
    MS_CHECK_HIP(hipMemsetAsync(out, 0, sizeof(int32_t), (hipStream_t)stream));
    if (total_host) *total_host = 0;
    return 0;
  }
  exclusive_scan_i32(in, n, out, total_host, tmp, (hipStream_t)stream);
  MS_CHECK_LAUNCH();
  return 0;
}

extern "C" int ms_radix_sort_pairs(const void* keys_in, const int32_t* values_in, void* keys_out,
                                   int32_t* values_out, int64_t n, int key_bytes, int begin_bit,
                                   int end_bit, void* tmp, size_t* tmp_bytes, void* stream) {
  MS_CHECK_ARG(n >= 0, "n < 0");
  MS_CHECK_ARG(key_bytes == 4 || key_bytes == 8, "key_bytes must be 4 or 8");
  MS_CHECK_ARG(begin_bit >= 0 && end_bit >= begin_bit && end_bit <= key_bytes * 8, "bad bit range");
  MS_CHECK_ARG(tmp_bytes != nullptr, "tmp_bytes is null");
  const size_t need = sort_tmp_layout(n, key_bytes).total;
  if (tmp == nullptr) { *tmp_bytes = need; return 0; }
  if (*tmp_bytes < need) { set_error("ms_radix_sort_pairs: tmp too small (%zu < %zu)", *tmp_bytes, need); return MS_ERR_TMP_TOO_SMALL; }
  if (n == 0) return 0;
  MS_CHECK_ARG(keys_in && values_in && keys_out && values_out, "null pointer");
  if (key_bytes == 4)
    radix_sort_pairs_impl<uint32_t>((const uint32_t*)keys_in, values_in, (uint32_t*)keys_out, values_out, n, begin_bit, end_bit, (char*)tmp, (hipStream_t)stream);
  else
    radix_sort_pairs_impl<uint64_t>((const uint64_t*)keys_in, values_in, (uint64_t*)keys_out, values_out, n, begin_bit, end_bit, (char*)tmp, (hipStream_t)stream);
  MS_CHECK_LAUNCH();
  return 0;
}

extern "C" int ms_depth_argsort(const void* depth, int64_t v, int depth16, double ndc_near, double ndc_far,
                               int dtype, uint32_t* out_sorted_keys, int32_t* out_order, void* tmp,
                               size_t* tmp_bytes, void* stream) {
  MS_CHECK_ARG(v >= 0, "v < 0");
  MS_CHECK_ARG(dtype == MS_F32 || dtype == MS_F64, "dtype must be MS_F32 or MS_F64");
  MS_CHECK_ARG(tmp_bytes != nullptr, "tmp_bytes is null");
  const size_t need = sort_tmp_layout(v, 4).total;
  if (tmp == nullptr) { *tmp_bytes = need; return 0; }
  if (*tmp_bytes < need) { set_error("ms_depth_argsort: tmp too small (%zu < %zu)", *tmp_bytes, need); return MS_ERR_TMP_TOO_SMALL; }
  if (v == 0) return 0;
  MS_CHECK_ARG(depth && out_sorted_keys && out_order, "null pointer");
  const int end_bit = depth16 ? 16 : 32;
  if (dtype == MS_F32)
    radix_sort_passes<uint32_t>(DepthPairs<float>{(const float*)depth, depth16, ndc_near, ndc_far, 0}, out_sorted_keys, out_order, v, 0, end_bit, (char*)tmp, (hipStream_t)stream);
  else
    radix_sort_passes<uint32_t>(DepthPairs<double>{(const double*)depth, depth16, ndc_near, ndc_far, 0}, out_sorted_keys, out_order, v, 0, end_bit, (char*)tmp, (hipStream_t)stream);
  MS_CHECK_LAUNCH();
  return 0;
}

extern "C" int ms_segmented_sort_pairs(const int32_t* keys_in, const int32_t* values_in, int32_t* keys_out,
                                       int32_t* values_out, int64_t n, const int64_t* start_offsets,
                                       const int64_t* end_offsets, int64_t num_segments, void* stream) {
  MS_CHECK_ARG(n >= 0 && num_segments >= 0, "negative size");
  if (n == 0 || num_segments == 0) return 0;
  MS_CHECK_ARG(keys_in && values_in && keys_out && values_out && start_offsets && end_offsets, "null pointer");
  copy_pairs_kernel<int32_t><<<dim3((unsigned)div_up(n, 256)), dim3(256), 0, (hipStream_t)stream>>>(
      keys_in, values_in, keys_out, values_out, n);
  segmented_rank_sort_kernel<<<dim3((unsigned)num_segments), dim3(256), 0, (hipStream_t)stream>>>(
      keys_in, values_in, keys_out, values_out, start_offsets, end_offsets);
  MS_CHECK_LAUNCH();
  return 0;
}

extern "C" int ms_find_ranges(const void* sorted_keys, int64_t k, int key_bytes, int tile_shift,
                              int64_t num_tiles, int32_t* out_ranges, void* stream) {
  MS_CHECK_ARG(k >= 0 && num_tiles >= 0, "negative size");
  MS_CHECK_ARG(key_bytes == 4 || key_bytes == 8, "key_bytes must be 4 or 8");
  MS_CHECK_ARG(out_ranges != nullptr || num_tiles == 0, "out_ranges is null");
  if (num_tiles > 0)
    MS_CHECK_HIP(hipMemsetAsync(out_ranges, 0, (size_t)num_tiles * 2 * sizeof(int32_t), (hipStream_t)stream));
  if (k == 0) return 0;
  MS_CHECK_ARG(sorted_keys != nullptr, "sorted_keys is null");
  const dim3 block(256), grid((unsigned)div_up(k, 256));
  if (key_bytes == 4)
    find_ranges_kernel<uint32_t><<<grid, block, 0, (hipStream_t)stream>>>((const uint32_t*)sorted_keys, k, nullptr, tile_shift, num_tiles, out_ranges);
  else
    find_ranges_kernel<uint64_t><<<grid, block, 0, (hipStream_t)stream>>>((const uint64_t*)sorted_keys, k, nullptr, tile_shift, num_tiles, out_ranges);
  MS_CHECK_LAUNCH();
  return 0;
}
```

taichi_splatting_amd/csrc/tile_sort.hip:

```cpp
#include "common.h"
#include "frame_internal.h"

namespace ms {

constexpr int TS_THREADS = 256;
constexpr int TS_WAVES = TS_THREADS / 64;
constexpr int TS_COST_LIMIT = 64;
constexpr int SMALL_R = 4, MID_R = 10, LONG_R = 20;

constexpr int TS_PER_WAVE = 256;
struct TsShared {
  uint32_t red[2 * TS_WAVES];
  uint32_t hist[256];
};
constexpr uint64_t TS_DECLINED = ~0ull;
constexpr int TS_REPORT_ABOVE = 16384;

__device__ __forceinline__ uint32_t ts_wave_min(uint32_t v) {
#pragma unroll
  for (int o = 32; o > 0; o >>= 1) { const uint32_t w = (uint32_t)__shfl_xor((int)v, o); v = w < v ? w : v; }
  return v;
}
__device__ __forceinline__ uint32_t ts_wave_max(uint32_t v) {
#pragma unroll
  for (int o = 32; o > 0; o >>= 1) { const uint32_t w = (uint32_t)__shfl_xor((int)v, o); v = w > v ? w : v; }
  return v;
}
__device__ __forceinline__ uint32_t ts_wave_or(uint32_t v) {
#pragma unroll
  for (int o = 32; o > 0; o >>= 1) v |= (uint32_t)__shfl_xor((int)v, o);
  return v;
}
__device__ __forceinline__ uint32_t ts_wave_and(uint32_t v) {
#pragma unroll
  for (int o = 32; o > 0; o >>= 1) v &= (uint32_t)__shfl_xor((int)v, o);
  return v;
}
__device__ __forceinline__ uint32_t ts_wave_sum(uint32_t v) {
#pragma unroll
  for (int o = 32; o > 0; o >>= 1) v += (uint32_t)__shfl_xor((int)v, o);
  return v;
}
__device__ __forceinline__ uint32_t ts_wave_scan(uint32_t v) {
  const int lane = threadIdx.x & 63;
#pragma unroll
  for (int o = 1; o < 64; o <<= 1) { const uint32_t w = (uint32_t)__shfl_up((int)v, o); if (lane >= o) v += w; }
  return v;
}

__device__ __forceinline__ uint32_t ts_block_exclusive(uint32_t v, uint32_t* red, uint32_t* total) {
  const int lane = threadIdx.x & 63, wave = threadIdx.x >> 6;
  const uint32_t inc = ts_wave_scan(v);
  __syncthreads();
  if (lane == 63) red[wave] = inc;
  __syncthreads();
  uint32_t before = 0, all = 0;
#pragma unroll
  for (int w = 0; w < TS_WAVES; ++w) { const uint32_t c = red[w]; if (w < wave) before += c; all += c; }
  *total = all;
  return before + inc - v;
}

__device__ void tile_radix_sort_global(uint64_t* srt, int32_t* o2p, uint64_t* alt,
                                       int64_t b, int n, TsShared& sh, uint32_t* wcnt) {
  const int t = threadIdx.x, lane = t & 63, wave = t >> 6;
  uint32_t kor = 0u, kand = 0xffffffffu;
  for (int i = t; i < n; i += TS_THREADS) {
    const uint32_t k = (uint32_t)srt[b + i];
    srt[b + i] = ((uint64_t)k << 32) | (uint32_t)o2p[b + i];
    kor |= k;
    kand &= k;
  }
  kor = ts_wave_or(kor);
  kand = ts_wave_and(kand);
  __syncthreads();
  if (lane == 0) { sh.red[wave] = kor; sh.red[TS_WAVES + wave] = kand; }
  __syncthreads();
  kor = 0u; kand = 0xffffffffu;
#pragma unroll
  for (int w = 0; w < TS_WAVES; ++w) { kor |= sh.red[w]; kand &= sh.red[TS_WAVES + w]; }
  const uint32_t vary = kor ^ kand;

  uint64_t* src = srt;
  uint64_t* dst = alt;
  for (int pass = 0; pass < 4; ++pass) {
    if (((vary >> (8 * pass)) & 0xffu) == 0u) continue;
    const int shift = 32 + 8 * pass;
    __syncthreads();
    sh.hist[t] = 0u;
    __syncthreads();
    for (int i = t; i < n; i += TS_THREADS) atomicAdd(&sh.hist[(uint32_t)(src[b + i] >> shift) & 0xffu], 1u);
    __syncthreads();
    uint32_t total;
    const uint32_t base = ts_block_exclusive(sh.hist[t], sh.red, &total);
    __syncthreads();
    sh.hist[t] = base;
    __syncthreads();
    for (int c = 0; c < n; c += TS_WAVES * TS_PER_WAVE) {
      for (int j = t; j < TS_WAVES * 256; j += TS_THREADS) wcnt[j] = 0u;
      __syncthreads();
      uint64_t p[TS_PER_WAVE / 64];
      uint32_t rank[TS_PER_WAVE / 64];
#pragma unroll
      for (int g = 0; g < TS_PER_WAVE / 64; ++g) {
        const int i = c + wave * TS_PER_WAVE + g * 64 + lane;
        const bool valid = i < n;
        p[g] = valid ? src[b + i] : 0ull;
        const uint32_t d = (uint32_t)(p[g] >> shift) & 0xffu;
        uint64_t peers = __ballot(valid);
#pragma unroll
        for (int bit = 0; bit < 8; ++bit) {
          const bool one = (d >> bit) & 1u;
          const uint64_t bal = __ballot(one);
          peers &= one ? bal : ~bal;
        }
        const uint64_t below = peers & ((1ull << lane) - 1ull);
        uint32_t prev = 0u;
        if (valid) prev = wcnt[wave * 256 + d];
        __builtin_amdgcn_wave_barrier();
        if (valid && below == 0ull) wcnt[wave * 256 + d] = prev + (uint32_t)__popcll(peers);
        __builtin_amdgcn_wave_barrier();
        rank[g] = prev + (uint32_t)__popcll(below);
      }
      __syncthreads();
      {
        uint32_t at = sh.hist[t];
#pragma unroll
        for (int w = 0; w < TS_WAVES; ++w) { const uint32_t cw = wcnt[w * 256 + t]; wcnt[w * 256 + t] = at; at += cw; }
        sh.hist[t] = at;
      }
      __syncthreads();
#pragma unroll
      for (int g = 0; g < TS_PER_WAVE / 64; ++g) {
        const int i = c + wave * TS_PER_WAVE + g * 64 + lane;
        if (i < n) dst[b + wcnt[wave * 256 + ((uint32_t)(p[g] >> shift) & 0xffu)] + rank[g]] = p[g];
      }
      __syncthreads();
    }
    uint64_t* const swap = src; src = dst; dst = swap;
  }
  __syncthreads();
  if (src == srt && vary == 0u) return;
  for (int i = t; i < n; i += TS_THREADS) o2p[b + i] = (int32_t)(uint32_t)src[b + i];
}

struct BucketMap {
  uint32_t kmin, top;
  float base, scale;
  int by_value;
  __device__ __forceinline__ uint32_t operator()(uint32_t k) const {
    const float x = by_value ? __uint_as_float(k) - base : (float)(k - kmin);
    const uint32_t bkt = (uint32_t)(x * scale);
    return bkt < top ? bkt : top;
  }
};

template <int R>
__device__ __forceinline__ bool tile_bucket_sort(uint64_t* __restrict__ srt, int32_t* __restrict__ o2p,
                                                 int64_t b, int n, uint64_t* pairs, uint32_t* cnt, TsShared& sh) {
  const int t = threadIdx.x, lane = t & 63, wave = t >> 6;
  uint32_t key[R], id[R];
  uint32_t kmin = 0xffffffffu, kmax = 0u;
#pragma unroll
  for (int r = 0; r < R; ++r) {
    const int i = t + TS_THREADS * r;
    key[r] = 0u; id[r] = 0u;
    if (i < n) {
      key[r] = (uint32_t)srt[b + i];
      id[r] = (uint32_t)o2p[b + i];
      kmin = key[r] < kmin ? key[r] : kmin;
      kmax = key[r] > kmax ? key[r] : kmax;
    }
  }
  kmin = ts_wave_min(kmin);
  kmax = ts_wave_max(kmax);
  if (lane == 0) { sh.red[wave] = kmin; sh.red[TS_WAVES + wave] = kmax; }
  __syncthreads();
#pragma unroll
  for (int w = 0; w < TS_WAVES; ++w) {
    kmin = sh.red[w] < kmin ? sh.red[w] : kmin;
    kmax = sh.red[TS_WAVES + w] > kmax ? sh.red[TS_WAVES + w] : kmax;
  }
  if (kmin == kmax) return true;

  const uint32_t nb = (uint32_t)n;
  BucketMap bucket;
  bucket.kmin = kmin;
  bucket.top = nb - 1u;
  bucket.by_value = kmin >= 0x00800000u && kmax < 0x7f800000u;
  bucket.base = __uint_as_float(kmin);
  bucket.scale = (float)nb / (__uint_as_float(kmax) - bucket.base);
  if (bucket.by_value && !(bucket.scale < 3.0e38f)) bucket.by_value = 0;
  if (!bucket.by_value) bucket.scale = (float)nb / (float)(kmax - kmin);

  for (uint32_t j = t; j < nb; j += TS_THREADS) cnt[j] = 0u;
  __syncthreads();
  uint32_t bkt[R], slot[R];
#pragma unroll
  for (int r = 0; r < R; ++r) {
    bkt[r] = 0u; slot[r] = 0u;
    if (t + TS_THREADS * r < n) {
      bkt[r] = bucket(key[r]);
      slot[r] = atomicAdd(&cnt[bkt[r]], 1u);
    }
  }
  __syncthreads();

  const uint32_t per = (nb + TS_THREADS - 1u) / TS_THREADS;
  const uint32_t j0 = t * per, j1 = j0 + per < nb ? j0 + per : nb;
  uint32_t mine = 0u, squares = 0u;
  for (uint32_t j = j0; j < j1; ++j) { const uint32_t c = cnt[j]; mine += c; squares += c * c; }
  const uint32_t inc = ts_wave_scan(mine);
  squares = ts_wave_sum(squares);
  if (lane == 63) { sh.red[wave] = inc; sh.red[TS_WAVES + wave] = squares; }
  __syncthreads();
  uint32_t run = inc - mine, cost = 0u;
#pragma unroll
  for (int w = 0; w < TS_WAVES; ++w) {
    if (w < wave) run += sh.red[w];
    cost += sh.red[TS_WAVES + w];
  }
  if (cost > (uint32_t)TS_COST_LIMIT * nb) return false;
  for (uint32_t j = j0; j < j1; ++j) { const uint32_t c = cnt[j]; cnt[j] = run; run += c; }
  __syncthreads();

#pragma unroll
  for (int r = 0; r < R; ++r)
    if (t + TS_THREADS * r < n) pairs[cnt[bkt[r]] + slot[r]] = ((uint64_t)key[r] << 32) | id[r];
  __syncthreads();

#pragma unroll
  for (int r = 0; r < R; ++r) {
    const int i = t + TS_THREADS * r;
    if (i < n) {
      const uint64_t p = pairs[i];
      const uint32_t g = bucket((uint32_t)(p >> 32));
      const uint32_t first = cnt[g], last = g + 1u < nb ? cnt[g + 1u] : nb;
      uint32_t rank = first;
      for (uint32_t m = first; m < last; ++m) rank += pairs[m] < p ? 1u : 0u;
      o2p[b + rank] = (int32_t)(uint32_t)p;
    }
  }
  return true;
}

template <int R>
__global__ void __launch_bounds__(TS_THREADS, R <= 4 ? 8 : 1)
tile_depth_sort_kernel(const int32_t* __restrict__ ranges, uint64_t* __restrict__ srt, int32_t* __restrict__ o2p,
                       uint64_t* __restrict__ alt, int lo, int hi, int32_t* __restrict__ run_stats) {
  constexpr int CAP = TS_THREADS * R;
  __shared__ uint64_t pairs[CAP];
  __shared__ uint32_t cnt[CAP];
  __shared__ TsShared sh;
  const int64_t tile = blockIdx.x;
  const int64_t b = ranges[2 * tile];
  const int n = ranges[2 * tile + 1] - (int32_t)b;
  if (n <= lo || n > hi) return;
  const bool sorted = tile_bucket_sort<R>(srt, o2p, b, n, pairs, cnt, sh);
  if (threadIdx.x == 0) {
    alt[b] = sorted ? 0ull : TS_DECLINED;
    if (!sorted && run_stats) atomicOr(run_stats + 2, 1);
  }
}

template <int R>
__global__ void __launch_bounds__(TS_THREADS)
tile_depth_sort_long_kernel(const int32_t* __restrict__ ranges, int64_t num_tiles, uint64_t* __restrict__ srt,
                            int32_t* __restrict__ o2p, uint64_t* __restrict__ alt, int lo, int32_t* __restrict__ run_stats,
                            int32_t* __restrict__ run_host) {
  constexpr int CAP = TS_THREADS * R;
  static_assert(CAP >= TS_WAVES * 256, "the bucket counters double as the bounded path's digit counters");
  __shared__ uint64_t pairs[CAP];
  __shared__ uint32_t cnt[CAP];
  __shared__ TsShared sh;
  __shared__ int32_t todo[TS_THREADS];
  __shared__ int32_t todo_count;
  const int64_t share = (num_tiles + gridDim.x - 1) / gridDim.x;
  const int64_t first = (int64_t)blockIdx.x * share;
  const int64_t last = first + share < num_tiles ? first + share : num_tiles;
  const bool any_declined = run_stats ? run_stats[2] != 0 : true;
  for (int64_t base = first; base < last; base += TS_THREADS) {
    __syncthreads();
    if (threadIdx.x == 0) todo_count = 0;
    __syncthreads();
    const int64_t mine = base + threadIdx.x;
    if (mine < last) {
      const int64_t mb = ranges[2 * mine];
      const int mn = ranges[2 * mine + 1] - (int32_t)mb;
      if (mn > lo) {
        todo[atomicAdd(&todo_count, 1)] = (int32_t)(mine - base);
        if (mn > TS_REPORT_ABOVE && run_host) *run_host = mn;
      }
      else if (any_declined && mn > 1 && alt[mb] == TS_DECLINED) todo[atomicAdd(&todo_count, 1)] = (int32_t)(mine - base) | (1 << 30);
    }
    __syncthreads();
    const int count = todo_count;
    for (int j = 0; j < count; ++j) {
      const int entry = todo[j];
      const int64_t tile = base + (entry & 0xffff);
      const int64_t b = ranges[2 * tile];
      const int n = ranges[2 * tile + 1] - (int32_t)b;
      bool sorted = false;
      if (n <= CAP && !(entry >> 30)) sorted = tile_bucket_sort<R>(srt, o2p, b, n, pairs, cnt, sh);
      if (!sorted) {
        __syncthreads();
        tile_radix_sort_global(srt, o2p, alt, b, n, sh, cnt);
      }
      __syncthreads();
    }
  }
}

void tile_depth_sort_launch(const int32_t* tile_ranges, int64_t num_tiles, uint64_t* sorted_keys, int32_t* overlap_to_point,
                            uint64_t* scratch, hipStream_t s, int32_t* run_stats, int32_t* run_host) {
  if (num_tiles <= 0) return;
  const dim3 per_tile((unsigned)num_tiles), block(TS_THREADS);
  tile_depth_sort_kernel<SMALL_R><<<per_tile, block, 0, s>>>(tile_ranges, sorted_keys, overlap_to_point, scratch, 1,
                                                            TS_THREADS * SMALL_R, run_stats);
  tile_depth_sort_kernel<MID_R><<<per_tile, block, 0, s>>>(tile_ranges, sorted_keys, overlap_to_point, scratch,
                                                          TS_THREADS * SMALL_R, TS_THREADS * MID_R, run_stats);
  const int64_t few = 2 * 256;
  tile_depth_sort_long_kernel<LONG_R><<<dim3((unsigned)(num_tiles < few ? num_tiles : few)), block, 0, s>>>(
      tile_ranges, num_tiles, sorted_keys, overlap_to_point, scratch, TS_THREADS * MID_R, run_stats, run_host);
}

}

using namespace ms;

extern "C" int ms_tile_depth_sort(const int32_t* tile_ranges, int64_t num_tiles, uint64_t* sorted_keys,
                                  int32_t* overlap_to_point, uint64_t* scratch, void* stream) {
  MS_CHECK_ARG(num_tiles >= 0 && num_tiles < (1ll << 31), "num_tiles out of range");
  if (num_tiles == 0) return 0;
  MS_CHECK_ARG(tile_ranges && sorted_keys && overlap_to_point && scratch, "null pointer");
  tile_depth_sort_launch(tile_ranges, num_tiles, sorted_keys, overlap_to_point, scratch, (hipStream_t)stream);
  MS_CHECK_LAUNCH();
  return 0;
}
```

Baseline: 1995 Msplats/s.

## Sort overlaps by 32-bit tile key with packed depth/id values

The direct mapper now emits a 32-bit tile-id key with a 64-bit value packing depth and splat index. It replaces the 64-bit key radix sort over tile and depth bits. The global sort covers only the tile bits, and the per-tile depth sort reads the packed pairs and writes overlap_to_point itself. This cuts key traffic in the global sort, at the cost of wider values and an extra write of o2p for tiles that were already uniform.

```diff
diff --git a/taichi_splatting_amd/csrc/frame.hip b/taichi_splatting_amd/csrc/frame.hip
--- a/taichi_splatting_amd/csrc/frame.hip
+++ b/taichi_splatting_amd/csrc/frame.hip
@@ -117,10 +117,10 @@
   L->split_scratch = keep_k.take(frame_uses_split(d) ? split_scratch_bytes(d->k_capacity, d->raster.tile_size, frame_split_params(d)) : 0);
   L->keep_k_bytes = keep_k.off;
 
-  L->keys = scratch_k.take(k * 8);
-  L->values = scratch_k.take(k * 4);
-  L->keys_sorted = scratch_k.take(k * 8);
-  L->tmp_k = scratch_k.take(sort_tmp_size(d->k_capacity, 8));
+  L->keys = scratch_k.take(k * 4);
+  L->values = scratch_k.take(k * 8);
+  L->keys_sorted = scratch_k.take(k * 4);
+  L->tmp_k = scratch_k.take(sort_tmp_size(d->k_capacity, 4, false, 8));
   L->scratch_k_bytes = scratch_k.off;
 }
 
@@ -329,8 +329,8 @@
   if (!d.projected_input && !colours_elsewhere) MS_TRY(frame_project_impl(desc, in, keep_n, false, true, stream, "ms_frame_map_raster"));
   if (d.n > 0 && d.k_capacity > 0) {
     MS_CHECK_ARG(keep_k && scratch_k, "null overlap buffers");
-    int32_t* values = (int32_t*)(sk + L.values);
     if (mapper_presort(d)) {
+      int32_t* values = (int32_t*)(sk + L.values);
       uint32_t* keys = (uint32_t*)(sk + L.keys);
       uint32_t* keys_sorted = (uint32_t*)(sk + L.keys_sorted);
       tile_emit_ordered_launch((const float*)(sn + L.ordered_points), (const int32_t*)(sn + L.order),
@@ -339,20 +339,20 @@
       sort_pairs_u32_dev_launch(keys, values, keys_sorted, o2p, d.k_capacity, counters + 1, g.tile_bits, sk + L.tmp_k, s);
       MS_TRY(find_ranges_dev_launch(keys_sorted, d.k_capacity, counters + 1, g.num_tiles, ranges, s, true));
     } else {
-      uint64_t* keys = (uint64_t*)(sk + L.keys);
-      uint64_t* keys_sorted = (uint64_t*)(sk + L.keys_sorted);
+      uint32_t* keys = (uint32_t*)(sk + L.keys);
+      uint64_t* values = (uint64_t*)(sk + L.values);
       const void* depth = d.projected_input ? in->depth : (const void*)(kn + L.depth);
       const float* points_f32 = d.dtype == MS_F64 ? (const float*)(sn + L.points7_f32)
                                                   : (const float*)(d.projected_input ? in->points7 : (const void*)(kn + L.points7));
       tile_emit_direct_launch(points_f32, depth, d.dtype, (const int32_t*)(sn + L.cum), d.n, g.w_pad, g.h_pad,
                               d.raster.tile_size, (float)d.raster.alpha_threshold, g.row_begin, g.row_end, d.depth16,
                               d.near_plane > 0.0 ? d.near_plane : 0.0, d.far_plane, counters + 1, keys, values, s);
-      sort_pairs_u64_dev_launch(keys, values, keys_sorted, o2p, d.k_capacity, counters + 1, 32, 32 + g.tile_bits,
-                                sk + L.tmp_k, s);
-      MS_TRY(find_ranges_u64_dev_launch(keys_sorted, d.k_capacity, counters + 1, g.num_tiles, ranges, s));
+      const TileSorted sorted = sort_tile_pairs_dev_launch(keys, values, d.k_capacity, counters + 1, g.tile_bits, sk + L.tmp_k, s);
+      MS_TRY(find_ranges_dev_launch(sorted.keys, d.k_capacity, counters + 1, g.num_tiles, ranges, s, true));
       const int64_t first_tile = (int64_t)g.row_begin * g.tiles_wide;
       const int64_t strip_tiles = (int64_t)(g.row_end > g.row_begin ? g.row_end - g.row_begin : 0) * g.tiles_wide;
-      tile_depth_sort_launch(ranges + 2 * first_tile, strip_tiles, keys_sorted, o2p, keys, s, counters + 3, in->longest_run_host);
+      tile_depth_sort_packed_launch(ranges + 2 * first_tile, strip_tiles, sorted.vals, o2p, sorted.free_vals, s, counters + 3,
+                                    in->longest_run_host);
     }
   }
   MS_CHECK_LAUNCH();
diff --git a/taichi_splatting_amd/csrc/frame_internal.h b/taichi_splatting_amd/csrc/frame_internal.h
--- a/taichi_splatting_amd/csrc/frame_internal.h
+++ b/taichi_splatting_amd/csrc/frame_internal.h
@@ -30,7 +30,7 @@
 }
 
 size_t scan_tmp_size(int64_t n);
-size_t sort_tmp_size(int64_t n, int key_bytes, bool adaptive = false);
+size_t sort_tmp_size(int64_t n, int key_bytes, bool adaptive = false, int val_bytes = 4);
 void exclusive_scan_launch(const int32_t* in, int64_t n, int32_t* out, int32_t* total_host, void* tmp, hipStream_t s,
                            int32_t* total_copy = nullptr);
 void depth_argsort_launch(const void* depth, int64_t n, int depth16, double ndc_near, double ndc_far, int dtype,
@@ -40,10 +40,13 @@
 int find_ranges_dev_launch(const uint32_t* sorted_keys, int64_t capacity, const int32_t* k_dev, int64_t num_tiles,
                            int32_t* out_ranges, hipStream_t s, bool zeroed = false);
 
-void sort_pairs_u64_dev_launch(const uint64_t* keys_in, const int32_t* vals_in, uint64_t* keys_out, int32_t* vals_out,
-                               int64_t capacity, const int32_t* n_dev, int begin_bit, int end_bit, char* tmp, hipStream_t s);
-int find_ranges_u64_dev_launch(const uint64_t* sorted_keys, int64_t capacity, const int32_t* k_dev, int64_t num_tiles,
-                               int32_t* out_ranges, hipStream_t s);
+struct TileSorted {
+  uint32_t* keys;
+  uint64_t* vals;
+  uint64_t* free_vals;
+};
+TileSorted sort_tile_pairs_dev_launch(uint32_t* keys, uint64_t* vals, int64_t capacity, const int32_t* n_dev, int end_bit,
+                                      char* tmp, hipStream_t s);
 
 void tile_count_launch(const float* points7, const int32_t* order, const uint32_t* cull_keys, int64_t v, int image_w,
                        int image_h, int tile_size, float alpha_threshold, int row_begin, int row_end,
@@ -58,11 +61,14 @@
                               hipStream_t s);
 void tile_emit_direct_launch(const float* points7, const void* depth, int dtype, const int32_t* cum, int64_t v, int image_w,
                              int image_h, int tile_size, float alpha_threshold, int row_begin, int row_end, int depth16,
-                             double ndc_near, double ndc_far, const int32_t* k_limit_dev, uint64_t* out_keys,
-                             int32_t* out_values, hipStream_t s);
+                             double ndc_near, double ndc_far, const int32_t* k_limit_dev, uint32_t* out_keys,
+                             uint64_t* out_values, hipStream_t s);
 
 void tile_depth_sort_launch(const int32_t* tile_ranges, int64_t num_tiles, uint64_t* sorted_keys, int32_t* overlap_to_point,
                             uint64_t* scratch, hipStream_t s, int32_t* run_stats = nullptr, int32_t* run_host = nullptr);
+void tile_depth_sort_packed_launch(const int32_t* tile_ranges, int64_t num_tiles, uint64_t* sorted_pairs,
+                                   int32_t* overlap_to_point, uint64_t* scratch, hipStream_t s, int32_t* run_stats,
+                                   int32_t* run_host);
 
 int project_fwd_launch(const void* position, const void* log_scaling, const void* rotation, const void* alpha_logit,
                        const void* T_camera_world, const void* projection, int image_w, int image_h, double near_plane,
diff --git a/taichi_splatting_amd/csrc/mapper.hip b/taichi_splatting_amd/csrc/mapper.hip
--- a/taichi_splatting_amd/csrc/mapper.hip
+++ b/taichi_splatting_amd/csrc/mapper.hip
@@ -172,12 +172,12 @@
   if (i < v) counts[i] = count;
 }
 
-template <typename T>
-__global__ void __launch_bounds__(256)
-tile_emit_direct_kernel(const float* __restrict__ points, const T* __restrict__ depth, const int32_t* __restrict__ cum,
-                        int64_t v, int image_w, int image_h, int tile_size, float alpha_threshold, int row_begin,
-                        int row_end, int depth16, double near_plane, double far_plane,
-                        const int32_t* __restrict__ k_limit, uint64_t* __restrict__ keys, int32_t* __restrict__ values) {
+template <typename T, bool SPLIT>
+__device__ __forceinline__ void emit_direct_body(const float* __restrict__ points, const T* __restrict__ depth,
+                                                 const int32_t* __restrict__ cum, int64_t v, int image_w, int image_h,
+                                                 int tile_size, float alpha_threshold, int row_begin, int row_end, int depth16,
+                                                 double near_plane, double far_plane, const int32_t* __restrict__ k_limit,
+                                                 void* __restrict__ out_keys, void* __restrict__ out_values) {
   const int64_t i = (int64_t)blockIdx.x * blockDim.x + threadIdx.x;
   if (k_limit && *k_limit == 0) return;
   const int64_t first = i < v ? (int64_t)cum[i] : 0;
@@ -192,9 +192,34 @@
     uint32_t dk = depth_key;
     int32_t who = (int32_t)i;
     if (from >= 0) { dk = (uint32_t)__builtin_amdgcn_readlane((int)depth_key, from); who = __builtin_amdgcn_readlane((int32_t)i, from); }
-    keys[o] = (tile_id << 32) | dk;
-    values[o] = who;
+    if constexpr (SPLIT) {
+      ((uint32_t*)out_keys)[o] = (uint32_t)tile_id;
+      ((uint64_t*)out_values)[o] = ((uint64_t)dk << 32) | (uint32_t)who;
+    } else {
+      ((uint64_t*)out_keys)[o] = (tile_id << 32) | dk;
+      ((int32_t*)out_values)[o] = who;
+    }
   });
+}
+
+template <typename T>
+__global__ void __launch_bounds__(256)
+tile_emit_direct_kernel(const float* __restrict__ points, const T* __restrict__ depth, const int32_t* __restrict__ cum,
+                        int64_t v, int image_w, int image_h, int tile_size, float alpha_threshold, int row_begin,
+                        int row_end, int depth16, double near_plane, double far_plane,
+                        const int32_t* __restrict__ k_limit, uint32_t* __restrict__ keys, uint64_t* __restrict__ values) {
+  emit_direct_body<T, true>(points, depth, cum, v, image_w, image_h, tile_size, alpha_threshold, row_begin, row_end, depth16,
+                            near_plane, far_plane, k_limit, keys, values);
+}
+
+template <typename T>
+__global__ void __launch_bounds__(256)
+tile_emit_keys64_kernel(const float* __restrict__ points, const T* __restrict__ depth, const int32_t* __restrict__ cum,
+                        int64_t v, int image_w, int image_h, int tile_size, float alpha_threshold, int row_begin,
+                        int row_end, int depth16, double near_plane, double far_plane, uint64_t* __restrict__ keys,
+                        int32_t* __restrict__ values) {
+  emit_direct_body<T, false>(points, depth, cum, v, image_w, image_h, tile_size, alpha_threshold, row_begin, row_end, depth16,
+                             near_plane, far_plane, nullptr, keys, values);
 }
 
 template <typename T>
@@ -237,8 +262,8 @@
 
 void tile_emit_direct_launch(const float* points7, const void* depth, int dtype, const int32_t* cum, int64_t v, int image_w,
                              int image_h, int tile_size, float alpha_threshold, int row_begin, int row_end, int depth16,
-                             double ndc_near, double ndc_far, const int32_t* k_limit_dev, uint64_t* out_keys,
-                             int32_t* out_values, hipStream_t s) {
+                             double ndc_near, double ndc_far, const int32_t* k_limit_dev, uint32_t* out_keys,
+                             uint64_t* out_values, hipStream_t s) {
   const dim3 grid((unsigned)div_up(v, 256)), block(256);
   if (dtype == MS_F64)
     tile_emit_direct_kernel<double><<<grid, block, 0, s>>>(points7, (const double*)depth, cum, v, image_w, image_h, tile_size,
@@ -323,9 +348,16 @@
   }
   if (v == 0) return 0;
   MS_CHECK_ARG(points7 && depth && cum && out_keys && out_values, "null pointer");
-  tile_emit_direct_launch(points7, depth, depth_dtype, cum, v, image_w, image_h, tile_size, alpha_threshold, tile_row_begin,
-                          tile_row_end, depth16, ndc_near > 0.0 ? ndc_near : 0.0, ndc_far, nullptr, out_keys, out_values,
-                          (hipStream_t)stream);
+  const dim3 grid((unsigned)div_up(v, 256)), block(256);
+  const double near = ndc_near > 0.0 ? ndc_near : 0.0;
+  if (depth_dtype == MS_F64)
+    tile_emit_keys64_kernel<double><<<grid, block, 0, (hipStream_t)stream>>>(points7, (const double*)depth, cum, v, image_w, image_h,
+                                                                             tile_size, alpha_threshold, tile_row_begin, tile_row_end,
+                                                                             depth16, near, ndc_far, out_keys, out_values);
+  else
+    tile_emit_keys64_kernel<float><<<grid, block, 0, (hipStream_t)stream>>>(points7, (const float*)depth, cum, v, image_w, image_h,
+                                                                            tile_size, alpha_threshold, tile_row_begin, tile_row_end,
+                                                                            depth16, near, ndc_far, out_keys, out_values);
   MS_CHECK_LAUNCH();
   return 0;
 }
diff --git a/taichi_splatting_amd/csrc/scan_sort.hip b/taichi_splatting_amd/csrc/scan_sort.hip
--- a/taichi_splatting_amd/csrc/scan_sort.hip
+++ b/taichi_splatting_amd/csrc/scan_sort.hip
@@ -172,12 +172,14 @@
 }
 
 template <typename KeyT> struct PlainPairs {
+  using val_type = int32_t;
   const KeyT* keys;
   const int32_t* vals;
   __device__ __forceinline__ KeyT key(int64_t i) const { return keys[i]; }
   __device__ __forceinline__ int32_t val(int64_t i) const { return vals[i]; }
 };
 template <typename T> struct DepthPairs {
+  using val_type = int32_t;
   const T* depth;
   int depth16;
   double near_plane, far_plane;
@@ -188,6 +190,14 @@
     return depth_sort_key(d, depth16, near_plane, far_plane);
   }
   __device__ __forceinline__ int32_t val(int64_t i) const { return (int32_t)i; }
+};
+
+struct TilePairs {
+  using val_type = uint64_t;
+  const uint32_t* keys;
+  const uint64_t* vals;
+  __device__ __forceinline__ uint32_t key(int64_t i) const { return keys[i]; }
+  __device__ __forceinline__ uint64_t val(int64_t i) const { return vals[i]; }
 };
 
 template <typename KeyT, typename Source, bool VARY = false>
@@ -279,17 +289,18 @@
   row_scan_body(hist, num_blocks, digit_totals);
 }
 
-template <typename KeyT> struct DownsweepShared {
+template <typename KeyT, typename ValT = int32_t> struct DownsweepShared {
   unsigned cnt[RS_WAVES][RS_RADIX];
   int scan[4];
   unsigned digit_shift[RS_RADIX];
   KeyT keys[RS_TILE];
-  int32_t vals[RS_TILE];
+  ValT vals[RS_TILE];
 };
 
 template <typename KeyT, bool FULL, typename Source>
-__device__ __forceinline__ void downsweep_block(DownsweepShared<KeyT>& sh, const Source src, KeyT* __restrict__ keys_out,
-                                                int32_t* __restrict__ vals_out, int64_t n, int shift, unsigned mask,
+__device__ __forceinline__ void downsweep_block(DownsweepShared<KeyT, typename Source::val_type>& sh, const Source src,
+                                                KeyT* __restrict__ keys_out,
+                                                typename Source::val_type* __restrict__ vals_out, int64_t n, int shift, unsigned mask,
                                                 const int32_t* __restrict__ hist_scanned,
                                                 const int32_t* __restrict__ digit_totals, int64_t num_blocks) {
   for (int i = threadIdx.x; i < RS_WAVES * RS_RADIX; i += RS_THREADS) (&sh.cnt[0][0])[i] = 0;
@@ -300,7 +311,7 @@
   const unsigned long long lanes_below = (1ull << lane) - 1ull;
 
   KeyT k[RS_ROUNDS];
-  int32_t v[RS_ROUNDS];
+  typename Source::val_type v[RS_ROUNDS];
   unsigned rank[RS_ROUNDS];
 
 #pragma unroll
@@ -387,11 +398,11 @@
 template <typename KeyT, typename Source>
 __global__ void __launch_bounds__(RS_THREADS)
 radix_downsweep_kernel(const Source src,
-                       KeyT* __restrict__ keys_out, int32_t* __restrict__ vals_out, int64_t n,
+                       KeyT* __restrict__ keys_out, typename Source::val_type* __restrict__ vals_out, int64_t n,
                        const int32_t* __restrict__ n_dev, int shift,
                        unsigned mask, const int32_t* __restrict__ hist_scanned,
                        const int32_t* __restrict__ digit_totals, int64_t num_blocks) {
-  __shared__ DownsweepShared<KeyT> sh;
+  __shared__ DownsweepShared<KeyT, typename Source::val_type> sh;
   if (n_dev) {
     n = *n_dev;
     if ((int64_t)blockIdx.x * RS_TILE >= n) return;
@@ -414,14 +425,14 @@
   size_t hist_off, scan_off, keys_off, vals_off, keys2_off, vals2_off, vary_off, total;
 };
 
-static SortTmp sort_tmp_layout(int64_t n, int key_bytes, bool adaptive = false) {
+static SortTmp sort_tmp_layout(int64_t n, int key_bytes, bool adaptive = false, int val_bytes = sizeof(int32_t)) {
   const int64_t blocks = div_up(n > 0 ? n : 1, RS_TILE);
   SortTmp t;
   size_t off = 0;
   t.hist_off = off; off += align_up((size_t)(RS_RADIX * blocks + 1) * sizeof(int32_t), 256);
   t.scan_off = off; off += align_up((size_t)RS_RADIX * sizeof(int32_t), 256);
   t.keys_off = off; off += align_up((size_t)n * key_bytes, 256);
-  t.vals_off = off; off += align_up((size_t)n * sizeof(int32_t), 256);
+  t.vals_off = off; off += align_up((size_t)n * val_bytes, 256);
   t.keys2_off = t.vals2_off = t.vary_off = off;
   if (adaptive) {
     t.keys2_off = off; off += align_up((size_t)n * key_bytes, 256);
@@ -634,37 +645,8 @@
   }
 }
 
-__global__ void __launch_bounds__(256)
-find_ranges2_u64_kernel(const uint64_t* __restrict__ keys, int64_t capacity, const int32_t* __restrict__ k_dev,
-                        int64_t num_tiles, int32_t* __restrict__ ranges) {
-  const int64_t i0 = ((int64_t)blockIdx.x * blockDim.x + threadIdx.x) * 2;
-  const int64_t k = k_dev ? (int64_t)*k_dev : capacity;
-  uint32_t t0 = 0xffffffffu, t1 = 0xffffffffu;
-  if (i0 + 1 < k) {
-    const uint4 a = *reinterpret_cast<const uint4*>(keys + i0);
-    t0 = a.y; t1 = a.w;
-  } else if (i0 < k) {
-    t0 = (uint32_t)(keys[i0] >> 32);
-  }
-  uint32_t t2 = (uint32_t)__shfl_down((int)t0, 1);
-  if ((threadIdx.x & 63) == 63) t2 = i0 + 2 < k ? (uint32_t)(keys[i0 + 2] >> 32) : 0xffffffffu;
-  if (i0 >= k) return;
-  if (i0 == 0 && (int64_t)t0 < num_tiles) ranges[(int64_t)t0 * 2 + 0] = 0;
-  const uint32_t t[3] = {t0, t1, t2};
-#pragma unroll
-  for (int j = 0; j < 2; ++j) {
-    const int64_t i = i0 + j;
-    if (i >= k) break;
-    const int64_t tile = t[j], next = (i + 1 < k) ? (int64_t)t[j + 1] : -1;
-    if (tile != next) {
-      if (tile < num_tiles) ranges[tile * 2 + 1] = (int32_t)(i + 1);
-      if (next >= 0 && next < num_tiles) ranges[next * 2 + 0] = (int32_t)(i + 1);
-    }
-  }
-}
-
 size_t scan_tmp_size(int64_t n) { return scan_tmp_bytes(n); }
-size_t sort_tmp_size(int64_t n, int key_bytes, bool adaptive) { return sort_tmp_layout(n, key_bytes, adaptive).total; }
+size_t sort_tmp_size(int64_t n, int key_bytes, bool adaptive, int val_bytes) { return sort_tmp_layout(n, key_bytes, adaptive, val_bytes).total; }
 
 void exclusive_scan_launch(const int32_t* in, int64_t n, int32_t* out, int32_t* total_host, void* tmp, hipStream_t s,
                            int32_t* total_copy) {
@@ -693,16 +675,29 @@
   return 0;
 }
 
-void sort_pairs_u64_dev_launch(const uint64_t* keys_in, const int32_t* vals_in, uint64_t* keys_out, int32_t* vals_out,
-                               int64_t capacity, const int32_t* n_dev, int begin_bit, int end_bit, char* tmp, hipStream_t s) {
-  radix_sort_passes<uint64_t>(PlainPairs<uint64_t>{keys_in, vals_in}, keys_out, vals_out, capacity, begin_bit, end_bit, tmp, s, n_dev);
-}
-
-int find_ranges_u64_dev_launch(const uint64_t* sorted_keys, int64_t capacity, const int32_t* k_dev, int64_t num_tiles,
-                               int32_t* out_ranges, hipStream_t s) {
-  if (capacity > 0)
-    find_ranges2_u64_kernel<<<dim3((unsigned)div_up(capacity, 512)), dim3(256), 0, s>>>(sorted_keys, capacity, k_dev, num_tiles, out_ranges);
-  return 0;
+TileSorted sort_tile_pairs_dev_launch(uint32_t* keys, uint64_t* vals, int64_t capacity, const int32_t* n_dev, int end_bit,
+                                      char* tmp, hipStream_t s) {
+  const int64_t blocks = div_up(capacity, RS_TILE);
+  const SortTmp lay = sort_tmp_layout(capacity, sizeof(uint32_t), false, sizeof(uint64_t));
+  int32_t* hist = (int32_t*)(tmp + lay.hist_off);
+  int32_t* digit_totals = (int32_t*)(tmp + lay.scan_off);
+  uint32_t* k_set[2] = {keys, (uint32_t*)(tmp + lay.keys_off)};
+  uint64_t* v_set[2] = {vals, (uint64_t*)(tmp + lay.vals_off)};
+  const int passes = (end_bit + 7) / 8;
+  const dim3 grid((unsigned)blocks), block(RS_THREADS);
+  const int base_bits = end_bit / passes, wide = end_bit % passes;
+  int shift = 0;
+  for (int p = 0; p < passes; ++p) {
+    const int bits = base_bits + (p < wide ? 1 : 0);
+    const unsigned mask = (1u << bits) - 1u;
+    const TilePairs src{k_set[p & 1], v_set[p & 1]};
+    radix_upsweep_kernel<uint32_t, TilePairs><<<grid, block, 0, s>>>(src, capacity, n_dev, shift, mask, hist, blocks);
+    radix_row_scan_kernel<<<dim3(RS_RADIX), dim3(SCAN_THREADS), 0, s>>>(hist, blocks, digit_totals);
+    radix_downsweep_kernel<uint32_t, TilePairs><<<grid, block, 0, s>>>(src, k_set[(p + 1) & 1], v_set[(p + 1) & 1], capacity, n_dev,
+                                                                       shift, mask, hist, digit_totals, blocks);
+    shift += bits;
+  }
+  return TileSorted{k_set[passes & 1], v_set[passes & 1], v_set[(passes + 1) & 1]};
 }
 
 }
diff --git a/taichi_splatting_amd/csrc/tile_sort.hip b/taichi_splatting_amd/csrc/tile_sort.hip
--- a/taichi_splatting_amd/csrc/tile_sort.hip
+++ b/taichi_splatting_amd/csrc/tile_sort.hip
@@ -61,13 +61,21 @@
   return before + inc - v;
 }
 
+template <bool PACKED>
+__device__ __forceinline__ uint64_t ts_load_pair(const uint64_t* __restrict__ srt, const int32_t* __restrict__ o2p, int64_t i) {
+  if constexpr (PACKED) return srt[i];
+  else return ((uint64_t)(uint32_t)srt[i] << 32) | (uint32_t)o2p[i];
+}
+
+template <bool PACKED>
 __device__ void tile_radix_sort_global(uint64_t* srt, int32_t* o2p, uint64_t* alt,
                                        int64_t b, int n, TsShared& sh, uint32_t* wcnt) {
   const int t = threadIdx.x, lane = t & 63, wave = t >> 6;
   uint32_t kor = 0u, kand = 0xffffffffu;
   for (int i = t; i < n; i += TS_THREADS) {
-    const uint32_t k = (uint32_t)srt[b + i];
-    srt[b + i] = ((uint64_t)k << 32) | (uint32_t)o2p[b + i];
+    const uint64_t p = ts_load_pair<PACKED>(srt, o2p, b + i);
+    if (!PACKED) srt[b + i] = p;
+    const uint32_t k = (uint32_t)(p >> 32);
     kor |= k;
     kand &= k;
   }
@@ -140,7 +148,7 @@
     uint64_t* const swap = src; src = dst; dst = swap;
   }
   __syncthreads();
-  if (src == srt && vary == 0u) return;
+  if (!PACKED && src == srt && vary == 0u) return;
   for (int i = t; i < n; i += TS_THREADS) o2p[b + i] = (int32_t)(uint32_t)src[b + i];
 }
 
@@ -155,8 +163,8 @@
   }
 };
 
-template <int R>
-__device__ __forceinline__ bool tile_bucket_sort(uint64_t* __restrict__ srt, int32_t* __restrict__ o2p,
+template <int R, bool PACKED>
+__device__ __forceinline__ bool tile_bucket_sort(const uint64_t* __restrict__ srt, int32_t* __restrict__ o2p,
                                                  int64_t b, int n, uint64_t* pairs, uint32_t* cnt, TsShared& sh) {
   const int t = threadIdx.x, lane = t & 63, wave = t >> 6;
   uint32_t key[R], id[R];
@@ -166,8 +174,9 @@
     const int i = t + TS_THREADS * r;
     key[r] = 0u; id[r] = 0u;
     if (i < n) {
-      key[r] = (uint32_t)srt[b + i];
-      id[r] = (uint32_t)o2p[b + i];
+      const uint64_t p = ts_load_pair<PACKED>(srt, o2p, b + i);
+      key[r] = (uint32_t)(p >> 32);
+      id[r] = (uint32_t)p;
       kmin = key[r] < kmin ? key[r] : kmin;
       kmax = key[r] > kmax ? key[r] : kmax;
     }
@@ -181,7 +190,14 @@
     kmin = sh.red[w] < kmin ? sh.red[w] : kmin;
     kmax = sh.red[TS_WAVES + w] > kmax ? sh.red[TS_WAVES + w] : kmax;
   }
-  if (kmin == kmax) return true;
+  if (kmin == kmax) {
+    if (PACKED) {
+#pragma unroll
+      for (int r = 0; r < R; ++r)
+        if (t + TS_THREADS * r < n) o2p[b + t + TS_THREADS * r] = (int32_t)id[r];
+    }
+    return true;
+  }
 
   const uint32_t nb = (uint32_t)n;
   BucketMap bucket;
@@ -244,10 +260,10 @@
   return true;
 }
 
-template <int R>
-__global__ void __launch_bounds__(TS_THREADS, R <= 4 ? 8 : 1)
-tile_depth_sort_kernel(const int32_t* __restrict__ ranges, uint64_t* __restrict__ srt, int32_t* __restrict__ o2p,
-                       uint64_t* __restrict__ alt, int lo, int hi, int32_t* __restrict__ run_stats) {
+template <int R, bool PACKED>
+__device__ __forceinline__ void tile_depth_sort_body(const int32_t* __restrict__ ranges, const uint64_t* __restrict__ srt,
+                                                     int32_t* __restrict__ o2p, uint64_t* __restrict__ alt, int lo, int hi,
+                                                     int32_t* __restrict__ run_stats) {
   constexpr int CAP = TS_THREADS * R;
   __shared__ uint64_t pairs[CAP];
   __shared__ uint32_t cnt[CAP];
@@ -256,7 +272,7 @@
   const int64_t b = ranges[2 * tile];
   const int n = ranges[2 * tile + 1] - (int32_t)b;
   if (n <= lo || n > hi) return;
-  const bool sorted = tile_bucket_sort<R>(srt, o2p, b, n, pairs, cnt, sh);
+  const bool sorted = tile_bucket_sort<R, PACKED>(srt, o2p, b, n, pairs, cnt, sh);
   if (threadIdx.x == 0) {
     alt[b] = sorted ? 0ull : TS_DECLINED;
     if (!sorted && run_stats) atomicOr(run_stats + 2, 1);
@@ -264,6 +280,20 @@
 }
 
 template <int R>
+__global__ void __launch_bounds__(TS_THREADS, R <= 4 ? 8 : 1)
+tile_depth_sort_kernel(const int32_t* __restrict__ ranges, const uint64_t* __restrict__ srt, int32_t* __restrict__ o2p,
+                       uint64_t* __restrict__ alt, int lo, int hi, int32_t* __restrict__ run_stats) {
+  tile_depth_sort_body<R, true>(ranges, srt, o2p, alt, lo, hi, run_stats);
+}
+
+template <int R>
+__global__ void __launch_bounds__(TS_THREADS, R <= 4 ? 8 : 1)
+tile_depth_sort_keyed_kernel(const int32_t* __restrict__ ranges, const uint64_t* __restrict__ srt, int32_t* __restrict__ o2p,
+                             uint64_t* __restrict__ alt, int lo, int hi, int32_t* __restrict__ run_stats) {
+  tile_depth_sort_body<R, false>(ranges, srt, o2p, alt, lo, hi, run_stats);
+}
+
+template <int R, bool PACKED>
 __global__ void __launch_bounds__(TS_THREADS)
 tile_depth_sort_long_kernel(const int32_t* __restrict__ ranges, int64_t num_tiles, uint64_t* __restrict__ srt,
                             int32_t* __restrict__ o2p, uint64_t* __restrict__ alt, int lo, int32_t* __restrict__ run_stats,
@@ -301,27 +331,46 @@
       const int64_t b = ranges[2 * tile];
       const int n = ranges[2 * tile + 1] - (int32_t)b;
       bool sorted = false;
-      if (n <= CAP && !(entry >> 30)) sorted = tile_bucket_sort<R>(srt, o2p, b, n, pairs, cnt, sh);
+      if (n <= CAP && !(entry >> 30)) sorted = tile_bucket_sort<R, PACKED>(srt, o2p, b, n, pairs, cnt, sh);
       if (!sorted) {
         __syncthreads();
-        tile_radix_sort_global(srt, o2p, alt, b, n, sh, cnt);
-      }
-      __syncthreads();
-    }
-  }
+        tile_radix_sort_global<PACKED>(srt, o2p, alt, b, n, sh, cnt);
+      }
+      __syncthreads();
+    }
+  }
+}
+
+template <bool PACKED>
+static void tile_depth_sort_launch_impl(const int32_t* tile_ranges, int64_t num_tiles, uint64_t* srt, int32_t* overlap_to_point,
+                                        uint64_t* scratch, hipStream_t s, int32_t* run_stats, int32_t* run_host) {
+  if (num_tiles <= 0) return;
+  const dim3 per_tile((unsigned)num_tiles), block(TS_THREADS);
+  if (PACKED) {
+    tile_depth_sort_kernel<SMALL_R><<<per_tile, block, 0, s>>>(tile_ranges, srt, overlap_to_point, scratch, 0,
+                                                              TS_THREADS * SMALL_R, run_stats);
+    tile_depth_sort_kernel<MID_R><<<per_tile, block, 0, s>>>(tile_ranges, srt, overlap_to_point, scratch,
+                                                            TS_THREADS * SMALL_R, TS_THREADS * MID_R, run_stats);
+  } else {
+    tile_depth_sort_keyed_kernel<SMALL_R><<<per_tile, block, 0, s>>>(tile_ranges, srt, overlap_to_point, scratch, 1,
+                                                                    TS_THREADS * SMALL_R, run_stats);
+    tile_depth_sort_keyed_kernel<MID_R><<<per_tile, block, 0, s>>>(tile_ranges, srt, overlap_to_point, scratch,
+                                                                  TS_THREADS * SMALL_R, TS_THREADS * MID_R, run_stats);
+  }
+  const int64_t few = 2 * 256;
+  tile_depth_sort_long_kernel<LONG_R, PACKED><<<dim3((unsigned)(num_tiles < few ? num_tiles : few)), block, 0, s>>>(
+      tile_ranges, num_tiles, srt, overlap_to_point, scratch, TS_THREADS * MID_R, run_stats, run_host);
 }
 
 void tile_depth_sort_launch(const int32_t* tile_ranges, int64_t num_tiles, uint64_t* sorted_keys, int32_t* overlap_to_point,
                             uint64_t* scratch, hipStream_t s, int32_t* run_stats, int32_t* run_host) {
-  if (num_tiles <= 0) return;
-  const dim3 per_tile((unsigned)num_tiles), block(TS_THREADS);
-  tile_depth_sort_kernel<SMALL_R><<<per_tile, block, 0, s>>>(tile_ranges, sorted_keys, overlap_to_point, scratch, 1,
-                                                            TS_THREADS * SMALL_R, run_stats);
-  tile_depth_sort_kernel<MID_R><<<per_tile, block, 0, s>>>(tile_ranges, sorted_keys, overlap_to_point, scratch,
-                                                          TS_THREADS * SMALL_R, TS_THREADS * MID_R, run_stats);
-  const int64_t few = 2 * 256;
-  tile_depth_sort_long_kernel<LONG_R><<<dim3((unsigned)(num_tiles < few ? num_tiles : few)), block, 0, s>>>(
-      tile_ranges, num_tiles, sorted_keys, overlap_to_point, scratch, TS_THREADS * MID_R, run_stats, run_host);
+  tile_depth_sort_launch_impl<false>(tile_ranges, num_tiles, sorted_keys, overlap_to_point, scratch, s, run_stats, run_host);
+}
+
+void tile_depth_sort_packed_launch(const int32_t* tile_ranges, int64_t num_tiles, uint64_t* sorted_pairs,
+                                   int32_t* overlap_to_point, uint64_t* scratch, hipStream_t s, int32_t* run_stats,
+                                   int32_t* run_host) {
+  tile_depth_sort_launch_impl<true>(tile_ranges, num_tiles, sorted_pairs, overlap_to_point, scratch, s, run_stats, run_host);
 }
 
 }
```

Result: no change. 1999 Msplats/s (median of 4 runs) (+0.2%).
